# Gabriel-SGama/Semantic-SuperPoint

Hardware: NVIDIA B200
Metric: loss-step pairs/s @240x320 B32 (higher is better)
Workload: dtype bf16x3 (hi/lo split bf16 on tcgen05, fp32 accumulate, fp32-grade)

## Files before the change

include/ssp_b200.h:

```cpp
#ifndef SSP_B200_H
#define SSP_B200_H
#include <stddef.h>
#include <stdint.h>
#ifdef __cplusplus
extern "C" {
#endif

int ssp_version(void);
const char* ssp_last_error(void);
int ssp_sm_count(void);

int ssp_warp_points(const float* pts , int P, const float* H , int B,
                    float* out , void* stream);
int ssp_warp_points_mask(const float* pts, int P, const float* H, int B, float shape_x, float shape_y,
                         float* out , uint8_t* keep , void* stream);
int ssp_warp_keypoints_f64(const double* kp , int K, const double* H , double W,
                           double Hh, double* out , uint8_t* keep , void* stream);

int ssp_inv_warp_image(const float* img , int B, int C, int H, int W, const float* Hinv ,
                       const float* xs, const float* ys, int mode, float* out , void* stream);

int ssp_valid_mask(int B, int H, int W, const float* Hinv, const float* xs, const float* ys, const uint8_t* kern,
                   int kh, int kw, int ax, int ay, float* out , void* stream);

int ssp_labels2d_to_3d(const float* labels , int B, int H, int W, int add_dustbin,
                       float* out , void* stream);
int ssp_cell_mask(const float* mask2d , int B, int H, int W, float* out , void* stream);
size_t ssp_detector_loss_ws_bytes(int B, int Hc, int Wc);
int ssp_detector_loss_fwd(const float* semi , const float* target, const float* mask, int B, int Hc,
                          int Wc, int fused2d, float* out3, void* ws, size_t ws_bytes, void* stream);
int ssp_detector_loss_bwd(const float* semi, const float* target, const float* mask, int B, int Hc, int Wc,
                          int fused2d, const float* fwd_out3, const float* gout , float* dsemi, void* stream);
int ssp_detector_loss_fwd_pair(const float* semi0, const float* target0, const float* mask0, const float* semi1,
                               const float* target1, const float* mask1, int B, int Hc, int Wc, int fused2d,
                               float* out3_0, float* out3_1, float* cellmask1, void* ws, size_t ws_bytes, void* stream);
int ssp_detector_loss_bwd_pair(const float* semi0, const float* target0, const float* mask0, const float* semi1,
                               const float* target1, const float* mask1, int B, int Hc, int Wc, int fused2d,
                               const float* fwd0, const float* fwd1, const float* gout0, const float* gout1,
                               float* dsemi0, float* dsemi1, void* stream);

int ssp_flatten_detection(const float* semi , int N, int Hc, int Wc, float* heat ,
                          void* stream);

int ssp_flatten_detection_masked(const float* semi , const float* mask , int N, int Hc,
                                 int Wc, float* heat , int* flag, void* stream);

int ssp_combine_heatmap(const float* heat , const float* mask ,
                        const float* Hinv , int I, int N, int H, int W, const float* xs, const float* ys,
                        float* out , void* stream);
int ssp_combine_heatmap_signed(const float* heat_signed , const float* Hinv , int I, int N, int H,
                               int W, const float* xs, const float* ys, const int* flag , float* out ,
                               void* stream);

size_t ssp_nms_ws_bytes(int I, int H, int W, int capacity);
int ssp_nms_fast(const float* heat , int I, int H, int W, float conf_thresh, int R, const uint8_t* stencil,
                 int border, int capacity, double* pts, int* counts_host, void* ws, size_t ws_bytes, void* stream);
int ssp_box_nms(const float* prob , int I, int H, int W, float min_prob, int R, const uint8_t* stencil,
                float* out , void* ws, size_t ws_bytes, void* stream);

int ssp_desc_geometry_nblocks(int B, int Nc);
int ssp_desc_geometry(const float* H , const float* mask_valid ,
                      const float* mask2d , int B,
                      int Hc, int Wc, int cell, float* wpts, float* mv_pad, double* mv_part ,
                      uint32_t* mvbits , void* stream);
int ssp_desc_pos_nblocks(int B, int Nc);
int ssp_desc_maxp(void);
int ssp_desc_pos_fwd(const float* D , const float* Dw, const float* wpts, const float* mv_pad, int B,
                     int Hc, int Wc, int Dch, int cell, float dist, float lamda, float mpos, float mneg,
                     double* partials, int* rowcol, float* rowdot, int* colcnt, int* colrow, float* coldot,
                     void* stream);
int ssp_desc_pos_planes_nblocks(int B, int Nc);
int ssp_desc_pos_fwd_planes(const void* Ahi, const void* Alo, const void* Bhi, const void* Blo, const float* wpts,
                            const float* mv_pad, int B, int Hc, int Wc, int cell, float dist, float lamda, float mpos,
                            float mneg, double* partials, int* rowcol, float* rowdot, int* colcnt, int* colrow,
                            float* coldot, void* stream);
int ssp_desc_dense_simt_nblocks(int B, int Nc);
int ssp_desc_dense_fwd_simt(const float* D, const float* Dw, const float* mv_pad, int B, int Hc, int Wc, int Dch,
                            float mneg, double* partials, uint32_t* bitsR, uint32_t* bitsC,
                            float* dbgS , void* stream);
int ssp_desc_pack(const float* src , const float* scale , int B, int Dch, int Nc,
                  void* hi , void* lo , void* stream);
int ssp_desc_pack2(const float* src0, const float* src1 , const float* scale, int B, int Dch, int Nc, void* hi0,
                   void* lo0, void* hi1, void* lo1, void* stream);
int ssp_desc_pack2_geometry(const float* src0, const float* src1, int B, int Dch, int Hc, int Wc, void* hi0, void* lo0 ,
                            void* hi1, void* lo1 , const float* H , const float* mask_valid ,
                            const float* mask2d , int cell, float* wpts, float* mv_pad, double* mv_part,
                            uint32_t* mvbits , void* stream);
int ssp_desc_dense_tc_nblocks(int B, int Nc);
int ssp_desc_dense_fwd_tc(const void* Ahi, const void* Alo, const void* Bhi, const void* Blo, const float* mv_pad,
                          const uint32_t* mvbits , int B, int Hc, int Wc, float mneg, double* partials,
                          uint32_t* bitsR, uint32_t* bitsC, float* dbgS, void* stream);
int ssp_desc_finalize(const double* pos_part, int npos, const double* neg_part, int nneg, const double* mv_part,
                      int nmv, int B, int Hc, int Wc, const int* overflow, float* out8,
                      const float* det0 , const float* det1, float lambda_loss, float* total , void* stream);
int ssp_desc_pair_mask(const float* wpts, int B, int Hc, int Wc, int cell, float dist, float* mask ,
                       void* stream);
int ssp_desc_alpha(const float* mv_pad, const float* g3 , const float* out8, int B,
                   int Nc_pad, float* alpha , float* srow ,
                   void* stream);
int ssp_desc_pos_coef(const int* rowcol, const float* rowdot, const int* colcnt, const int* colrow, const float* coldot,
                      const uint32_t* bitsR, const float* mv_pad, const float* g3, float gscale, int gmode,
                      const float* out8, int B, int Nc_pad, float lamda, float mpos, float* rowcoef, int* colrow_sorted,
                      float* colcoef, float* alpha_out, float* srow_out, uint32_t* bitsC_out, int Nc, void* stream);
int ssp_step_bwd_prologue(const float* semi0, const float* labels0, const float* mask0, const float* semi1,
                          const float* labels1, const float* mask1, int B, int Hc, int Wc, const float* fwd0 ,
                          const float* fwd1, const float* gout , float* dsemi0, float* dsemi1,
                          const int* rowcol, const float* rowdot, const int* colcnt, const int* colrow, const float* coldot,
                          const uint32_t* bitsR, const float* mv_pad, const float* g3, float gscale, int gmode,
                          const float* out8, float lamda, float mpos, float* rowcoef, int* colrow_sorted, float* colcoef,
                          float* alpha_out, float* srow_out, uint32_t* bitsC_out, void* stream);
int ssp_desc_pos_apply(const int* rowcol, const float* rowcoef, const int* colrow, const float* colcoef, const float* D,
                       const float* Dw, int B, int Dch, int Nc, int which , float* dD, float* dDw,
                       void* stream);
int ssp_desc_bits_gemm_simt(const uint32_t* bits, const float* src , const float* colscale,
                            const float* rowscale, const int* plist, const float* pcoef, const float* possrc, int B,
                            int Dch, int Nc, float* out , void* stream);
int ssp_desc_bits_gemm_tc_planes(const uint32_t* bits, const void* Bhi, const void* Blo, const float* rowscale,
                                 const int* plist, const float* pcoef, const void* pos_hi, const void* pos_lo, int B,
                                 int Nc, float* out , void* stream);
int ssp_desc_bits_gemm_tc_pair(const uint32_t* bits0, const void* Bhi0, const void* Blo0, const float* rowscale0,
                               const int* plist0, const float* pcoef0, const void* pos_hi0, const void* pos_lo0,
                               float* out0, const uint32_t* bits1, const void* Bhi1, const void* Blo1,
                               const float* rowscale1, const int* plist1, const float* pcoef1, const void* pos_hi1,
                               const void* pos_lo1, float* out1, int B, int Nc, void* stream);

size_t ssp_sem_ce_ws_bytes(int B, int C, int H, int W, int upsampled);
int ssp_sem_ce_fwd(const float* logits , const long long* labels, int B, int C, int H, int W,
                   int ignore_index, float* lse2 ,
                   float* out3, void* ws, size_t ws_bytes, void* stream);
int ssp_sem_ce_bwd(const float* logits, const long long* labels, const float* lse2, int B, int C, int H, int W,
                   int ignore_index, const float* out3, const float* gout ,
                   float* dlogits , void* stream);
int ssp_sem_ce_up8(const float* logits_lr, const long long* labels, int B, int C, int Hc, int Wc, int ignore_index,
                   float* gsum, float* out3, void* ws, size_t ws_bytes, void* stream);
int ssp_sem_ce_up8_bwd(const float* gsum, const float* out3, const float* gout, int B, int C, int Hc, int Wc,
                       float* dlogits , void* stream);

int ssp_sample_desc(const float* coarse, const double* pts, int K, int D, int Hc, int Wc, int cell, float* desc,
                    void* stream);
int ssp_nn_match(const float* desc1 , const float* desc2 , int D, int K1, int K2,
                 unsigned long long* best1 , unsigned long long* best2 , void* stream);

int ssp_transpose_batched(const float* src , int B, int rows, int cols, float* dst ,
                          void* stream);
int ssp_sparse_desc_loss_fwd(const float* Dt, const float* Dwt, const int* ia, const int* ib, int B, int Nc, int Dch, int K,
                             int Kn, float lamda, float mpos, float mneg, float* dots, float* stats, float* out3,
                             void* stream);
int ssp_sparse_desc_loss_bwd(const float* Dt, const float* Dwt, const int* ia, const int* ib, const float* dots,
                             const float* stats, const float* g3 , int B, int Nc, int Dch, int K, int Kn,
                             float lamda, float mpos, float mneg, float* dDt, float* dDwt, void* stream);
int ssp_sparse_sample(const float* mat_H , int B, int Hc, int Wc, int K, int nper, unsigned long long* state,
                      int* ia, int* ib, int* M , void* stream);
int ssp_sparse_finalize(const int* M , int B, float* out3, const float* det0, const float* det1,
                        float lambda_loss, float* total , void* stream);

size_t ssp_warp_labels_ws_bytes(int B, int H, int W);
int ssp_warp_labels(const float* pnts, const int* counts, int B, int Pmax, int H, int W, const float* Hpix, int bilinear,
                    float* labels, float* res, float* labels_bi , float* warped, int* kept, void* ws,
                    size_t ws_bytes, void* stream);

size_t ssp_xchg_bytes(void);
int ssp_xchg_max_ranks(void);
int ssp_xchg_alloc(void** buf, void* ipc_handle64_host);
int ssp_xchg_open(const void* ipc_handle64_host, void** peer_buf);
int ssp_xchg_close(void* peer_buf);
int ssp_xchg_free(void* buf);
int ssp_xchg_status(const void* local_buf, void* stream);
int ssp_loss_exchange(const void* const* bufs_host , int rank, int world,
                      float* det0, float* det1, float* desc8, float* sem0, float* sem1, int B_local, int Hc, int Wc,
                      float lambda_loss, float* total ,
                      double timeout_s, void* stream);

int ssp_debug_trace(void* buf);
int ssp_debug_trace_cap(void);

#ifdef __cplusplus
}
#endif
#endif
```

semantic-superpoint_b200/_lib.py:

```python
import ctypes
import os
import threading

import torch

from . import build as _build

_c = ctypes
_P = _c.c_void_p
_I = _c.c_int
_F = _c.c_float
_D = _c.c_double
_Z = _c.c_size_t

SIGNATURES = {
    "ssp_version": (_I, []),
    "ssp_last_error": (_c.c_char_p, []),
    "ssp_sm_count": (_I, []),
    "ssp_warp_points": (_I, [_P, _I, _P, _I, _P, _P]),
    "ssp_warp_points_mask": (_I, [_P, _I, _P, _I, _F, _F, _P, _P, _P]),
    "ssp_warp_keypoints_f64": (_I, [_P, _I, _P, _D, _D, _P, _P, _P]),
    "ssp_inv_warp_image": (_I, [_P, _I, _I, _I, _I, _P, _P, _P, _I, _P, _P]),
    "ssp_valid_mask": (_I, [_I, _I, _I, _P, _P, _P, _P, _I, _I, _I, _I, _P, _P]),
    "ssp_labels2d_to_3d": (_I, [_P, _I, _I, _I, _I, _P, _P]),
    "ssp_cell_mask": (_I, [_P, _I, _I, _I, _P, _P]),
    "ssp_detector_loss_ws_bytes": (_Z, [_I, _I, _I]),
    "ssp_detector_loss_fwd": (_I, [_P, _P, _P, _I, _I, _I, _I, _P, _P, _Z, _P]),
    "ssp_detector_loss_bwd": (_I, [_P, _P, _P, _I, _I, _I, _I, _P, _P, _P, _P]),
    "ssp_detector_loss_fwd_pair": (_I, [_P, _P, _P, _P, _P, _P, _I, _I, _I, _I, _P, _P, _P, _P, _Z, _P]),
    "ssp_detector_loss_bwd_pair": (_I, [_P, _P, _P, _P, _P, _P, _I, _I, _I, _I, _P, _P, _P, _P, _P, _P, _P]),
    "ssp_flatten_detection": (_I, [_P, _I, _I, _I, _P, _P]),
    "ssp_flatten_detection_masked": (_I, [_P, _P, _I, _I, _I, _P, _P, _P]),
    "ssp_combine_heatmap": (_I, [_P, _P, _P, _I, _I, _I, _I, _P, _P, _P, _P]),
    "ssp_combine_heatmap_signed": (_I, [_P, _P, _I, _I, _I, _I, _P, _P, _P, _P, _P]),
    "ssp_nms_ws_bytes": (_Z, [_I, _I, _I, _I]),
    "ssp_nms_fast": (_I, [_P, _I, _I, _I, _F, _I, _P, _I, _I, _P, _P, _P, _Z, _P]),
    "ssp_box_nms": (_I, [_P, _I, _I, _I, _F, _I, _P, _P, _P, _Z, _P]),
    "ssp_desc_geometry_nblocks": (_I, [_I, _I]),
    "ssp_desc_geometry": (_I, [_P, _P, _P, _I, _I, _I, _I, _P, _P, _P, _P, _P]),
    "ssp_desc_pos_nblocks": (_I, [_I, _I]),
    "ssp_desc_maxp": (_I, []),
    "ssp_desc_pos_fwd": (_I, [_P, _P, _P, _P, _I, _I, _I, _I, _I, _F, _F, _F, _F, _P, _P, _P, _P, _P, _P, _P]),
    "ssp_desc_pos_planes_nblocks": (_I, [_I, _I]),
    "ssp_desc_pos_fwd_planes": (_I, [_P, _P, _P, _P, _P, _P, _I, _I, _I, _I, _F, _F, _F, _F, _P, _P, _P, _P, _P, _P, _P]),
    "ssp_desc_dense_simt_nblocks": (_I, [_I, _I]),
    "ssp_desc_dense_fwd_simt": (_I, [_P, _P, _P, _I, _I, _I, _I, _F, _P, _P, _P, _P, _P]),
    "ssp_desc_pack": (_I, [_P, _P, _I, _I, _I, _P, _P, _P]),
    "ssp_desc_pack2": (_I, [_P, _P, _P, _I, _I, _I, _P, _P, _P, _P, _P]),
    "ssp_desc_pack2_geometry": (_I, [_P, _P, _I, _I, _I, _I, _P, _P, _P, _P, _P, _P, _P, _I, _P, _P, _P, _P, _P]),
    "ssp_desc_dense_tc_nblocks": (_I, [_I, _I]),
    "ssp_desc_dense_fwd_tc": (_I, [_P, _P, _P, _P, _P, _P, _I, _I, _I, _F, _P, _P, _P, _P, _P]),
    "ssp_desc_finalize": (_I, [_P, _I, _P, _I, _P, _I, _I, _I, _I, _P, _P, _P, _P, _F, _P, _P]),
    "ssp_desc_pair_mask": (_I, [_P, _I, _I, _I, _I, _F, _P, _P]),
    "ssp_desc_alpha": (_I, [_P, _P, _P, _I, _I, _P, _P, _P]),
    "ssp_desc_pos_coef": (_I, [_P, _P, _P, _P, _P, _P, _P, _P, _F, _I, _P, _I, _I, _F, _F, _P, _P, _P, _P, _P, _P, _I, _P]),
    "ssp_step_bwd_prologue": (_I, [_P] * 6 + [_I] * 3 + [_P] * 5 + [_P] * 8 + [_F, _I, _P, _F, _F] + [_P] * 7),
    "ssp_desc_pos_apply": (_I, [_P, _P, _P, _P, _P, _P, _I, _I, _I, _I, _P, _P, _P]),
    "ssp_desc_bits_gemm_simt": (_I, [_P, _P, _P, _P, _P, _P, _P, _I, _I, _I, _P, _P]),
    "ssp_desc_bits_gemm_tc_planes": (_I, [_P, _P, _P, _P, _P, _P, _P, _P, _I, _I, _P, _P]),
    "ssp_desc_bits_gemm_tc_pair": (_I, [_P] * 18 + [_I, _I, _P]),
    "ssp_sem_ce_ws_bytes": (_Z, [_I, _I, _I, _I, _I]),
    "ssp_sem_ce_fwd": (_I, [_P, _P, _I, _I, _I, _I, _I, _P, _P, _P, _Z, _P]),
    "ssp_sem_ce_bwd": (_I, [_P, _P, _P, _I, _I, _I, _I, _I, _P, _P, _P, _P]),
    "ssp_sem_ce_up8": (_I, [_P, _P, _I, _I, _I, _I, _I, _P, _P, _P, _Z, _P]),
    "ssp_sem_ce_up8_bwd": (_I, [_P, _P, _P, _I, _I, _I, _I, _P, _P]),
    "ssp_sample_desc": (_I, [_P, _P, _I, _I, _I, _I, _I, _P, _P]),
    "ssp_nn_match": (_I, [_P, _P, _I, _I, _I, _P, _P, _P]),
    "ssp_transpose_batched": (_I, [_P, _I, _I, _I, _P, _P]),
    "ssp_sparse_desc_loss_fwd": (_I, [_P, _P, _P, _P, _I, _I, _I, _I, _I, _F, _F, _F, _P, _P, _P, _P]),
    "ssp_sparse_desc_loss_bwd": (_I, [_P, _P, _P, _P, _P, _P, _P, _I, _I, _I, _I, _I, _F, _F, _F, _P, _P, _P]),
    "ssp_sparse_sample": (_I, [_P, _I, _I, _I, _I, _I, _P, _P, _P, _P, _P]),
    "ssp_sparse_finalize": (_I, [_P, _I, _P, _P, _P, _F, _P, _P]),
    "ssp_warp_labels_ws_bytes": (_Z, [_I, _I, _I]),
    "ssp_warp_labels": (_I, [_P, _P, _I, _I, _I, _I, _P, _I, _P, _P, _P, _P, _P, _P, _Z, _P]),
    "ssp_debug_trace": (_I, [_P]),
    "ssp_debug_trace_cap": (_I, []),
    "ssp_xchg_bytes": (_Z, []),
    "ssp_xchg_max_ranks": (_I, []),
    "ssp_xchg_alloc": (_I, [_c.POINTER(_P), _P]),
    "ssp_xchg_open": (_I, [_P, _c.POINTER(_P)]),
    "ssp_xchg_close": (_I, [_P]),
    "ssp_xchg_free": (_I, [_P]),
    "ssp_xchg_status": (_I, [_P, _P]),
    "ssp_loss_exchange": (_I, [_c.POINTER(_P), _I, _I, _P, _P, _P, _P, _P, _I, _I, _I, _F, _P, _D, _P]),
}

_lib = None
_lock = threading.Lock()
launch_count = 0


def lib_path():
    return _build.LIB_PATH


def load(build_if_missing=True):
    global _lib
    with _lock:
        if _lib is not None:
            return _lib
        path = _build.LIB_PATH
        if not os.path.exists(path):
            if not build_if_missing:
                raise RuntimeError("libssp_b200.so is missing: run `python -c 'import __graft_entry__ as g; g.build()'`")
            _build.build_library()
        lib = ctypes.CDLL(path)
        for name, (res, args) in SIGNATURES.items():
            fn = getattr(lib, name)
            fn.restype = res
            fn.argtypes = args
        _lib = lib
        return _lib


def check(rc, what):
    if rc != 0:
        msg = load().ssp_last_error()
        raise RuntimeError("%s failed (code %d): %s" % (what, rc, msg.decode() if msg else ""))


KERNELS_PER_CALL = {"ssp_nms_fast": 5, "ssp_box_nms": 4, "ssp_detector_loss_fwd": 2, "ssp_detector_loss_fwd_pair": 2,
                    "ssp_sem_ce_fwd": 2, "ssp_sem_ce_up8": 2}
kernel_count = 0
_prof = None


def profile_begin():
    global _prof
    _prof = {}


def profile_end():
    global _prof
    torch.cuda.synchronize()
    out = {k: (len(v), sum(a.elapsed_time(b) for a, b in v)) for k, v in _prof.items()}
    _prof = None
    return out


def call(name, *args):
    global launch_count, kernel_count
    launch_count += 1
    kernel_count += KERNELS_PER_CALL.get(name, 1)
    fn = getattr(load(), name)
    if _prof is None:
        check(fn(*args), name)
        return
    e0, e1 = torch.cuda.Event(enable_timing=True), torch.cuda.Event(enable_timing=True)
    e0.record()
    rc = fn(*args)
    e1.record()
    _prof.setdefault(name, []).append((e0, e1))
    check(rc, name)


def ptr(t):
    return None if t is None else _c.c_void_p(t.data_ptr())


def stream_of(t):
    return _c.c_void_p(torch.cuda.current_stream(t.device).cuda_stream)


def require_cuda(*tensors):
    for t in tensors:
        if t is not None and not t.is_cuda:
            raise RuntimeError(
                "ssp_b200 has no CPU path: got a %s tensor; move inputs to a CUDA device (sm_100a)" % t.device
            )


def f32c(t, device=None):
    if device is not None and t.device != torch.device(device):
        t = t.to(device)
    if t.dtype != torch.float32:
        t = t.float()
    t = t.contiguous()
    if t.data_ptr() % 16:
        t = t.clone()
    return t
```

semantic-superpoint_b200/csrc/desc_tc.cu:

```cuda
#include "desc_common.cuh"
#include "tc_ptx.cuh"
#include <algorithm>
#include <cstdlib>

#define TRACE_CAP 4096
#ifdef SSP_TRACE
__device__ long long* g_trace_buf = nullptr;
__device__ int g_trace_roles = 0xF;
#define TR_DECL(role) long long* tr_ = (g_trace_buf && ((g_trace_roles >> (role)) & 1)) ? g_trace_buf + ((size_t)blockIdx.x * 4 + (role)) * TRACE_CAP : nullptr; int trn_ = 0
#define TR_ONLY(cond) do { if (!(cond)) tr_ = nullptr; } while (0)
#define TR(tag) do { if (tr_ && trn_ < TRACE_CAP) tr_[trn_++] = (clock64() << 8) | (long long)(tag); } while (0)
#else
#define TR_DECL(role) do { } while (0)
#define TR_ONLY(cond) do { } while (0)
#define TR(tag) do { } while (0)
#endif

namespace {

constexpr int BM = 128;
constexpr int BN = 256;
constexpr int KD = 256;
constexpr int KC = 64;
constexpr int NKC = KD / KC;
constexpr int CHUNK_BYTES = BM * KC * 2;
constexpr int FWD_THREADS = 320;
constexpr int BAR_BYTES = 1024;

template <int P> struct FwdCfg {
  static constexpr int A_BYTES = P * NKC * CHUNK_BYTES;
  static constexpr int STAGE_BYTES = P * CHUNK_BYTES;
  static constexpr int NSTAGE = (P == 1) ? 10 : 3;
  static constexpr int B_BYTES = NSTAGE * STAGE_BYTES;
  static constexpr int SMEM = A_BYTES + B_BYTES + BAR_BYTES + 1024;
};

__device__ __forceinline__ uint8_t* align1024(uint8_t* p) {
  return reinterpret_cast<uint8_t*>((reinterpret_cast<uintptr_t>(p) + 1023) & ~(uintptr_t)1023);
}

template <bool BITS>
__device__ __forceinline__ void epi_chunk(const uint32_t (&v)[32], const float4 (&mq)[8], float mneg, uint64_t& su2,
                                          uint64_t& sw2, uint32_t& rowword) {
  const uint64_t mneg2 = tc::pack2(mneg, mneg);
  uint32_t eb[32];
#pragma unroll
  for (int i = 0; i < 16; ++i) {
    const uint64_t e2 = tc::sub2(mneg2, tc::pack2(__uint_as_float(v[2 * i]), __uint_as_float(v[2 * i + 1])));
    float e0, e1;
    tc::unpack2(e2, e0, e1);
    const uint64_t n2 = tc::pack2(fmaxf(-e0, 0.f), fmaxf(-e1, 0.f));
    su2 = tc::add2(su2, n2);
    const float4 m = mq[i >> 1];
    sw2 = tc::fma2(n2, (i & 1) ? tc::pack2(m.z, m.w) : tc::pack2(m.x, m.y), sw2);
    eb[2 * i] = __float_as_uint(e0);
    eb[2 * i + 1] = __float_as_uint(e1);
  }
  if (BITS) {
    uint32_t w = 0;
#pragma unroll
    for (int pos = 31; pos >= 0; --pos) {
      const int j = ((pos & 15) << 1) | (pos >> 4);
      w = __funnelshift_l(eb[j], w, 1);
    }
    rowword = w;
  }
}

__device__ __forceinline__ double f32_to_f64_bits(float f) {
  const uint32_t u = __float_as_uint(f);
  const uint32_t e = (u >> 23) & 0xffu;
  const unsigned long long sign = (unsigned long long)(u & 0x80000000u) << 32;
  unsigned long long d;
  if (e == 0u) d = sign;
  else if (e == 0xffu) d = sign | (0x7ffull << 52) | ((unsigned long long)(u & 0x7fffffu) << 29);
  else d = sign | ((unsigned long long)(e + 896u) << 52) | ((unsigned long long)(u & 0x7fffffu) << 29);
  return __longlong_as_double((long long)d);
}

template <int P, bool BITS>
__global__ void __launch_bounds__(FWD_THREADS, 1)
desc_dense_fwd_tc_kernel(const __grid_constant__ CUtensorMap tmA, const __grid_constant__ CUtensorMap tmB,
                         const __grid_constant__ CUtensorMap tmBl, const float* __restrict__ mv_pad, const uint32_t* __restrict__ mvbits, DescGeom g, int n_last,
                         double* __restrict__ partials, uint32_t* __restrict__ bitsR, float* __restrict__ dbgS) {
  using Cfg = FwdCfg<P>;
  constexpr int NSTAGE = Cfg::NSTAGE;
  extern __shared__ uint8_t smem_raw[];
  uint8_t* smem = align1024(smem_raw);
  uint8_t* sA = smem;
  uint8_t* sB = sA + Cfg::A_BYTES;
  uint64_t* bars = reinterpret_cast<uint64_t*>(sB + Cfg::B_BYTES);
  uint64_t* a_full = bars;
  uint64_t* a_empty = a_full + NKC;
  uint64_t* b_full = a_empty + NKC;
  uint64_t* b_empty = b_full + NSTAGE;
  uint64_t* t_full = b_empty + NSTAGE;
  uint64_t* t_empty = t_full + 2;
  uint32_t* tmem_ptr = reinterpret_cast<uint32_t*>(t_empty + 2);

  const int warp = threadIdx.x >> 5, lane = threadIdx.x & 31;
  const int MP = g.Nc_pad / (2 * BM), NT = g.Nc_pad / BN;
  const uint32_t cta_rank = tc::cluster_ctarank();
  const bool leader = cta_rank == 0;
  const int ncluster = gridDim.x >> 1, cid = blockIdx.x >> 1;
  const long long T = (long long)g.B * MP * NT;
  const int it0 = (int)(T * cid / ncluster), it1 = (int)(T * (cid + 1) / ncluster);

  if (warp == 8 && lane == 0) {
    tc::prefetch_tmap(&tmA);
    tc::prefetch_tmap(&tmB);
    tc::prefetch_tmap(&tmBl);
  }
  if (warp == 9) {
    if (lane == 0) {
      for (int k = 0; k < NKC; ++k) { tc::mbar_init(a_full + k, 1); tc::mbar_init(a_empty + k, 1); }
      for (int s = 0; s < NSTAGE; ++s) { tc::mbar_init(b_full + s, 1); tc::mbar_init(b_empty + s, 1); }
      for (int s = 0; s < 2; ++s) { tc::mbar_init(t_full + s, 1); tc::mbar_init(t_empty + s, 16); }
      tc::fence_barrier_init();
    }
    __syncwarp();
    tc::tmem_alloc2(tmem_ptr, 512);
  }
  tc::fence_before_sync();
  tc::cluster_sync_all();
  tc::fence_after_sync();
  const uint32_t tmem_base = *tmem_ptr;

  if (warp == 8) {
    {
      TR_DECL(1);
      TR_ONLY(lane == 0);
      const bool el = tc::elect_one();
      int prev_key = -1, stage_it = 0, nkeys = 0;
      for (int it = it0; it < it1; ++it) {
        const int key = it / NT, nt = it - key * NT;
        const int b = key / MP, mp = key - b * MP;
        const int row_base = b * g.Nc_pad;
        const bool newkey = key != prev_key;
        const bool last = nt == NT - 1;
        const int half = (last ? n_last : BN) >> 1;
        for (int kc = 0; kc < NKC; ++kc) {
          if (newkey) {
            TR(10);
            if (nkeys > 0) tc::mbar_wait(a_empty + kc, (uint32_t)((nkeys - 1) & 1));
            TR(11);
            if (el) {
              if (leader) tc::mbar_expect_tx(a_full + kc, 2 * P * CHUNK_BYTES);
              tc::tma_load_3d_2sm(&tmA, a_full + kc, sA + kc * P * CHUNK_BYTES, kc * KC, row_base + (2 * mp + (int)cta_rank) * BM, 0);
            }
          }
          {
            const int s = stage_it % NSTAGE;
            const uint32_t ph = (stage_it / NSTAGE) & 1;
            ++stage_it;
            TR(12);
            tc::mbar_wait(b_empty + s, ph ^ 1);
            TR(13);
            if (el) {
              if (leader) tc::mbar_expect_tx(b_full + s, 2 * P * half * KC * 2);
              tc::tma_load_3d_2sm(last ? &tmBl : &tmB, b_full + s, sB + s * Cfg::STAGE_BYTES, kc * KC,
                                  row_base + nt * BN + (int)cta_rank * half, 0);
            }
          }
        }
        if (newkey) { prev_key = key; ++nkeys; }
      }
    }
    __syncwarp();
  } else if (warp == 9) {
    if (leader) {
      TR_DECL(0);
      TR_ONLY(lane == 0);
      const bool el = tc::elect_one();
      if (tmem_base != 0u) __trap();
      const uint32_t sA_u = tc::smem_u32(sA), sB_u = tc::smem_u32(sB);
      int prev_key = -1, stage_it = 0, tcount = 0, nkeys = 0;
      for (int it = it0; it < it1; ++it, ++tcount) {
        const int key = it / NT, nt = it - key * NT;
        const bool newkey = key != prev_key;
        if (newkey) { prev_key = key; ++nkeys; }
        const bool last_of_key = (it + 1 == it1) || ((it + 1) / NT != key);
        const int ncols = nt == NT - 1 ? n_last : BN;
        const uint32_t idesc = tc::idesc_bf16_f32(2 * BM, ncols, 0, 0);
        const int as = tcount & 1;
        const uint32_t aph = (tcount >> 1) & 1;
        TR(2);
        tc::mbar_wait(t_empty + as, aph ^ 1);
        TR(3);
        tc::fence_after_sync();
        const uint32_t d_tmem = as * BN;
        uint32_t first = 1;
        for (int kc = 0; kc < NKC; ++kc) {
          if (newkey) {
            TR(1);
            tc::mbar_wait(a_full + kc, (uint32_t)((nkeys - 1) & 1));
            TR(8);
          }
          {
            const int s = stage_it % NSTAGE;
            const uint32_t ph = (stage_it / NSTAGE) & 1;
            ++stage_it;
            TR(4);
            tc::mbar_wait(b_full + s, ph);
            TR(5);
            tc::fence_after_sync();
            const uint64_t da_hi = tc::smem_desc_sw128(sA_u + (kc * P) * CHUNK_BYTES, 16, 1024);
            const uint64_t db_hi = tc::smem_desc_sw128(sB_u + s * Cfg::STAGE_BYTES, 16, 1024);
            if (el) {
              tc::mma2_ss_x4(d_tmem, da_hi, db_hi, idesc, first ? 0u : 1u);
              if (P == 2) {
                const uint64_t da_lo = tc::smem_desc_sw128(sA_u + (kc * P + 1) * CHUNK_BYTES, 16, 1024);
                const uint64_t db_lo = tc::smem_desc_sw128(sB_u + s * Cfg::STAGE_BYTES + (ncols >> 1) * (KC * 2), 16, 1024);
                tc::mma2_ss_x4(d_tmem, da_lo, db_hi, idesc, 1u);
                tc::mma2_ss_x4(d_tmem, da_hi, db_lo, idesc, 1u);
              }
              tc::mma2_commit_mc(b_empty + s, (uint16_t)0x3);
            }
            first = 0;
            TR(6);
          }
          if (last_of_key && el) tc::mma2_commit_mc(a_empty + kc, (uint16_t)0x3);
        }
        if (el) tc::mma2_commit_mc(t_full + as, (uint16_t)0x3);
        __syncwarp();
      }
    }
    __syncwarp();
  } else {
    const int q = warp & 3, half = warp >> 2;
    const int NW = g.Nc_pad / 32;
    const bool fold = mvbits != nullptr;
    int tcount = 0;
    double su_all = 0.0, sw_all = 0.0;
    TR_DECL(2 + (warp == 7 ? 1 : 0));
    TR_ONLY((warp == 0 || warp == 7) && lane == 0);
    for (int it = it0; it < it1; ++it, ++tcount) {
      const int key = it / NT, nt = it - key * NT;
      const int b = key / MP, mp = key - b * MP;
      const int row_base = b * g.Nc_pad;
      const int m0 = (2 * mp + (int)cta_rank) * BM;
      const int row = m0 + q * 32 + lane;
      const int ncols = nt == NT - 1 ? n_last : BN;
      const int ch0 = half * 4, ch1 = min((ncols + 31) >> 5, ch0 + 4);
      const int as = tcount & 1;
      const uint32_t aph = (tcount >> 1) & 1;
      float4 mq[8];
      if (ch0 < ch1) {
        const float4* mvq = reinterpret_cast<const float4*>(mv_pad + (size_t)row_base + nt * BN + ch0 * 32);
#pragma unroll
        for (int j4 = 0; j4 < 8; ++j4) mq[j4] = __ldg(mvq + j4);
      }
      TR(30);
      tc::mbar_wait(t_full + as, aph);
      TR(31);
      tc::fence_after_sync();
      uint64_t su2 = 0ull, sw2 = 0ull;
#pragma unroll 1
      for (int ch = ch0; ch < ch1; ++ch) {
        const int cbase = nt * BN + ch * 32;
        uint32_t v[32];
        tc::tmem_ld32(tmem_base + ((uint32_t)(q * 32) << 16) + as * BN + ch * 32, v);
        float4 mnext[8];
        if (ch + 1 < ch1) {
          const float4* mvq = reinterpret_cast<const float4*>(mv_pad + (size_t)row_base + cbase + 32);
#pragma unroll
          for (int j4 = 0; j4 < 8; ++j4) mnext[j4] = __ldg(mvq + j4);
        }
        tc::tmem_ld_wait();
        if (ch * 32 + 32 > ncols) {
#pragma unroll
          for (int j = 16; j < 32; ++j) v[j] = 0u;
        }
        uint32_t rowword = 0;
        epi_chunk<BITS>(v, mq, g.mneg, su2, sw2, rowword);
        if (BITS) {
          if (fold) rowword &= __ldg(mvbits + (size_t)b * NW + cbase / 32);
          bitsR[((size_t)b * NW + cbase / 32) * g.Nc_pad + row] = rowword;
        }
        if (dbgS && row < g.Nc) {
#pragma unroll
          for (int j = 0; j < 32; ++j)
            if (cbase + j < g.Nc) dbgS[((size_t)b * g.Nc + row) * g.Nc + cbase + j] = __uint_as_float(v[j]);
        }
        if (ch + 1 < ch1) {
#pragma unroll
          for (int j4 = 0; j4 < 8; ++j4) mq[j4] = mnext[j4];
        }
      }
      tc::fence_before_sync();
      __syncwarp();
      if (lane == 0) tc::mbar_arrive_leader(t_empty + as);
      TR(32);
      float sa, sb, wa, wb;
      tc::unpack2(su2, sa, sb);
      tc::unpack2(sw2, wa, wb);
      su_all += f32_to_f64_bits(sa + sb);
      sw_all += f32_to_f64_bits(wa + wb);
    }
    su_all = warp_sum_d(su_all);
    sw_all = warp_sum_d(sw_all);
    if (lane == 0) {
      const size_t slot = ((size_t)blockIdx.x * 8 + warp) * 2;
      partials[slot] = su_all;
      partials[slot + 1] = sw_all;
    }
  }

  tc::fence_before_sync();
  tc::cluster_sync_all();
  if (warp == 9) {
    tc::fence_after_sync();
    tc::tmem_dealloc2(tmem_base, 512);
  }
}

__global__ void __launch_bounds__(256)
desc_bits_transpose_kernel(const uint32_t* __restrict__ bitsR, uint32_t* __restrict__ bitsC, int NW, int NWv, int Nc_pad) {
  const int lane = threadIdx.x & 31, warp = threadIdx.x >> 5;
  const int rw = blockIdx.x, b = blockIdx.y;
  const int rl = ((lane & 15) << 1) | (lane >> 4);
  for (int cw0 = warp; cw0 < NW; cw0 += 32) {
    uint32_t w[4];
#pragma unroll
    for (int u = 0; u < 4; ++u) {
      const int cw = cw0 + 8 * u;
      w[u] = (cw < NWv && rw < NWv) ? __ldg(bitsR + ((size_t)b * NW + cw) * Nc_pad + rw * 32 + rl) : 0u;
    }
#pragma unroll
    for (int u = 0; u < 4; ++u) {
      const int cw = cw0 + 8 * u;
      if (cw >= NW) break;
      bitsC[((size_t)b * NW + rw) * Nc_pad + cw * 32 + rl] = warp_transpose32(w[u], lane);
    }
  }
}

constexpr int KT = 128;
constexpr int BG_PLANE_BYTES = KT * 128;
constexpr int BG_N = 128;
constexpr int BG_THREADS = 576;
constexpr int BG_W_EPI = 8, BG_W_TMA = 16, BG_W_MMA = 17;
constexpr int BG_NS = 4;
constexpr int BG_ACOLS = KT / 2;

constexpr int BG_PF = 4;
constexpr int BG_WRING_BYTES = 2 * BG_PF * 4 * BM * 4;

template <int P> struct BgCfg {
  static constexpr int STAGE_BYTES = P * BG_PLANE_BYTES;
  static constexpr int SMEM = BG_NS * STAGE_BYTES + BAR_BYTES + BG_WRING_BYTES + 1024;
};

struct BgJob {
  const uint32_t* bits;
  const float* rowscale;
  const int* plist;
  const float* pcoef;
  const uint4* pos_hi;
  const uint4* pos_lo;
  float* out;
};

template <int P>
__global__ void __launch_bounds__(BG_THREADS, 1)
desc_bits_gemm_tc_kernel(const __grid_constant__ CUtensorMap tm0, const __grid_constant__ CUtensorMap tm1, BgJob job0,
                         BgJob job1, int njobs, int B, int Nc, int Nc_pad) {
  using Cfg = BgCfg<P>;
  constexpr int NS = BG_NS;
  static_assert(256 + BG_ACOLS * NS <= 512, "TMEM A ring does not fit");
  extern __shared__ uint8_t smem_raw[];
  uint8_t* smem = align1024(smem_raw);
  uint64_t* bars = reinterpret_cast<uint64_t*>(smem + NS * Cfg::STAGE_BYTES);
  uint64_t* b_full = bars;
  uint64_t* a_full = b_full + NS;
  uint64_t* s_free = a_full + NS;
  uint64_t* d_full = s_free + NS;
  uint64_t* d_empty = d_full + 2;
  uint32_t* tmem_ptr = reinterpret_cast<uint32_t*>(d_empty + 2);
  uint32_t* wring = reinterpret_cast<uint32_t*>(smem + NS * Cfg::STAGE_BYTES + BAR_BYTES);

  const int warp = threadIdx.x >> 5, lane = threadIdx.x & 31;
  const int MP = Nc_pad / (2 * BM), NK = (Nc + KT - 1) / KT, NW = Nc_pad / 32;
  const int NKS = (Nc + 15) / 16;
  const uint32_t cta_rank = tc::cluster_ctarank();
  const bool leader = cta_rank == 0;
  const int ncluster = gridDim.x >> 1, cid = blockIdx.x >> 1;
  const int T = B * njobs * MP * 2;
  constexpr uint32_t A_COL0 = 256;

  auto decode = [&](int it, int& b, int& jb, int& mp, int& dh) {
    dh = it & 1;
    int t = it >> 1;
    mp = t % MP;
    t /= MP;
    jb = t % njobs;
    b = t / njobs;
  };

  if (warp == BG_W_TMA && lane == 0) {
    tc::prefetch_tmap(&tm0);
    if (njobs > 1) tc::prefetch_tmap(&tm1);
  }
  if (warp == BG_W_MMA) {
    if (lane == 0) {
      for (int s = 0; s < NS; ++s) { tc::mbar_init(b_full + s, 1); tc::mbar_init(a_full + s, 8); tc::mbar_init(s_free + s, 1); }
      for (int s = 0; s < 2; ++s) { tc::mbar_init(d_full + s, 1); tc::mbar_init(d_empty + s, 16); }
      tc::fence_barrier_init();
    }
    __syncwarp();
    tc::tmem_alloc2(tmem_ptr, 512);
  }
  tc::fence_before_sync();
  tc::cluster_sync_all();
  tc::fence_after_sync();
  const uint32_t tmem_base = *tmem_ptr;

  if (warp == BG_W_TMA) {
    {
      TR_DECL(1);
      TR_ONLY(lane == 0);
      const bool el = tc::elect_one();
      int st_it = 0;
      for (int it = cid; it < T; it += ncluster) {
        int b, jb, mp, dh;
        decode(it, b, jb, mp, dh);
        const CUtensorMap* m = jb ? &tm1 : &tm0;
        for (int kc = 0; kc < NK; ++kc, ++st_it) {
          const int s = st_it % NS;
          const uint32_t ph = (st_it / NS) & 1;
          TR(12);
          tc::mbar_wait(s_free + s, ph ^ 1);
          TR(13);
          if (el) {
            if (leader) tc::mbar_expect_tx(b_full + s, 2 * Cfg::STAGE_BYTES);
            tc::tma_load_3d_2sm(m, b_full + s, smem + s * Cfg::STAGE_BYTES, dh * BG_N + (int)cta_rank * 64, b * Nc_pad + kc * KT, 0);
          }
        }
      }
    }
    __syncwarp();
  } else if (warp == BG_W_MMA) {
    if (leader) {
      TR_DECL(0);
      TR_ONLY(lane == 0);
      const bool el = tc::elect_one();
      if (tmem_base != 0u) __trap();
      constexpr uint32_t idesc = tc::idesc_bf16_f32(2 * BM, BG_N, 0, 1);
      const uint32_t smem_u = tc::smem_u32(smem);
      int st_it = 0, tcount = 0;
      for (int it = cid; it < T; it += ncluster, ++tcount) {
        const int as = tcount & 1;
        const uint32_t aph = (tcount >> 1) & 1;
        TR(2);
        tc::mbar_wait(d_empty + as, aph ^ 1);
        TR(3);
        tc::fence_after_sync();
        const uint32_t d_tmem = as * BG_N;
        uint32_t first = 1;
        for (int kc = 0; kc < NK; ++kc, ++st_it) {
          const int s = st_it % NS;
          const uint32_t ph = (st_it / NS) & 1;
          TR(4);
          tc::mbar_wait(b_full + s, ph);
          TR(5);
          tc::mbar_wait(a_full + s, ph);
          TR(7);
          tc::fence_after_sync();
          const int nks = min(KT / 16, NKS - kc * (KT / 16));
          for (int p = 0; p < P; ++p) {
            const uint64_t db = tc::smem_desc_sw128(smem_u + s * Cfg::STAGE_BYTES + p * BG_PLANE_BYTES, BG_PLANE_BYTES, 1024);
            for (int j = 0; j < nks; ++j) {
              if (el) tc::mma2_ts(d_tmem, A_COL0 + s * BG_ACOLS + 8 * j, db + (uint64_t)(128 * j), idesc, first ? 0u : 1u);
              first = 0;
            }
          }
          if (el) tc::mma2_commit_mc(s_free + s, (uint16_t)0x3);
          TR(6);
        }
        if (el) tc::mma2_commit_mc(d_full + as, (uint16_t)0x3);
        __syncwarp();
      }
    }
    __syncwarp();
  } else if (warp < BG_W_EPI) {
    const int q = warp & 3, set = warp >> 2;
    TR_DECL(2);
    TR_ONLY(warp == 0 && lane == 0);
    auto expand_words = [&](uint32_t w0, uint32_t w1, uint32_t (&r)[32]) {
#pragma unroll
      for (int i = 0; i < 15; ++i) {
        r[i] = (w0 << (14 - i)) & 0x40004000u;
        r[16 + i] = (w1 << (14 - i)) & 0x40004000u;
      }
      r[15] = (w0 >> 1) & 0x40004000u;
      r[31] = (w1 >> 1) & 0x40004000u;
    };
    auto expand_stage = [&](int st_it, const uint32_t (&w)[4]) {
      const int s = st_it % NS;
      const uint32_t ph = (st_it / NS) & 1;
      uint32_t r[32];
      expand_words(w[0], w[1], r);
      TR(20);
      tc::mbar_wait(s_free + s, ph ^ 1);
      TR(21);
      tc::fence_after_sync();
      const uint32_t t0 = tmem_base + ((uint32_t)(q * 32) << 16) + A_COL0 + s * BG_ACOLS;
      tc::tmem_st32(t0, r);
      expand_words(w[2], w[3], r);
      tc::tmem_st32(t0 + 32, r);
      tc::tmem_st_wait();
      tc::fence_before_sync();
      __syncwarp();
      if (lane == 0) tc::mbar_arrive_leader(a_full + s);
      TR(23);
    };
    constexpr int PF = BG_PF;
    uint32_t* myring = wring + (size_t)set * PF * 4 * BM + (q * 32 + lane);
    int itB = cid, kcB = set;
    const uint32_t* pB = nullptr;
    bool newitem = true;
    auto fetch = [&](int slot) {
      while (itB < T && kcB >= NK) { kcB -= NK; itB += ncluster; newitem = true; }
      if (itB < T) {
        if (newitem) {
          int b, jb, mp, dh;
          decode(itB, b, jb, mp, dh);
          const int row = (2 * mp + (int)cta_rank) * BM + q * 32 + lane;
          pB = (jb ? job1.bits : job0.bits) + (size_t)b * NW * Nc_pad + row;
          newitem = false;
        }
#pragma unroll
        for (int u = 0; u < 4; ++u) tc::cp_async4(myring + (slot * 4 + u) * BM, pB + (size_t)(4 * kcB + u) * Nc_pad);
        kcB += 2;
      }
      tc::cp_async_commit();
    };
#pragma unroll
    for (int u = 0; u < PF; ++u) fetch(u);
    const int nitems = cid < T ? (T - cid + ncluster - 1) / ncluster : 0;
    const int total = nitems * NK;
    for (int g0 = set; g0 < total; g0 += 2 * PF) {
#pragma unroll
      for (int u = 0; u < PF; ++u) {
        if (g0 + 2 * u < total) {
          tc::cp_async_wait<PF - 1>();
          uint32_t w[4];
#pragma unroll
          for (int v = 0; v < 4; ++v) w[v] = myring[(u * 4 + v) * BM];
          expand_stage(g0 + 2 * u, w);
          fetch(u);
        }
      }
    }
    tc::cp_async_wait<0>();
  } else {
    const int q = warp & 3, chalf = (warp - BG_W_EPI) >> 2;
    int tcount = 0;
    TR_DECL(3);
    TR_ONLY(warp == BG_W_EPI && lane == 0);
    for (int it = cid; it < T; it += ncluster, ++tcount) {
      int b, jb, mp, dh;
      decode(it, b, jb, mp, dh);
      const BgJob& J = jb ? job1 : job0;
      const int row = (2 * mp + (int)cta_rank) * BM + q * 32 + lane;
      const bool row_ok = row < Nc;
      float rs = 0.5f;
      if (J.rowscale && row_ok) rs *= J.rowscale[(size_t)b * Nc_pad + row];
      const int* pl = J.plist ? J.plist + ((size_t)b * Nc_pad + row) * DESC_MAXP : nullptr;
      const float* pcf = J.plist ? J.pcoef + ((size_t)b * Nc_pad + row) * DESC_MAXP : nullptr;
      int npos = 0;
      if (pl && row_ok) {
#pragma unroll
        for (int n = 0; n < DESC_MAXP; ++n)
          if (pl[n] >= 0) npos = n + 1;
      }
      const int nmax = __reduce_max_sync(0xffffffffu, npos);
      const int as = tcount & 1;
      const uint32_t aph = (tcount >> 1) & 1;
      TR(30);
      tc::mbar_wait(d_full + as, aph);
      TR(31);
      tc::fence_after_sync();
      auto add_partner = [&](int n, int ch, float (&val)[32]) {
        int pc = n < npos ? pl[n] : -1;
        if (pc < 0) return;
        float pf = pcf[n];
        const size_t o = (((size_t)b * Nc_pad + pc) * KD + dh * BG_N + ch * 32) >> 3;
#pragma unroll
        for (int u = 0; u < 4; ++u) {
          const uint4 h = __ldg(J.pos_hi + o + u);
          const uint32_t hw[4] = {h.x, h.y, h.z, h.w};
          uint32_t lw[4] = {0u, 0u, 0u, 0u};
          if (J.pos_lo) {
            const uint4 l = __ldg(J.pos_lo + o + u);
            lw[0] = l.x; lw[1] = l.y; lw[2] = l.z; lw[3] = l.w;
          }
#pragma unroll
          for (int i = 0; i < 4; ++i) {
            float e0 = __uint_as_float(hw[i] << 16) + __uint_as_float(lw[i] << 16);
            float e1 = __uint_as_float(hw[i] & 0xffff0000u) + __uint_as_float(lw[i] & 0xffff0000u);
            val[u * 8 + 2 * i] = fmaf(pf, e0, val[u * 8 + 2 * i]);
            val[u * 8 + 2 * i + 1] = fmaf(pf, e1, val[u * 8 + 2 * i + 1]);
          }
        }
      };
#pragma unroll 1
      for (int ch = chalf * 2; ch < chalf * 2 + 2; ++ch) {
        uint32_t v[32];
        tc::tmem_ld32(tmem_base + ((uint32_t)(q * 32) << 16) + as * BG_N + ch * 32, v);
        tc::tmem_ld_wait();
        if (row_ok) {
          float val[32];
#pragma unroll
          for (int j = 0; j < 32; ++j) val[j] = __uint_as_float(v[j]) * rs;
#pragma unroll 1
          for (int n = 0; n < nmax; ++n) add_partner(n, ch, val);
          float* o = J.out + ((size_t)b * KD + dh * BG_N + ch * 32) * Nc + row;
#pragma unroll
          for (int j = 0; j < 32; ++j) o[(size_t)j * Nc] = val[j];
        }
      }
      tc::fence_before_sync();
      __syncwarp();
      if (lane == 0) tc::mbar_arrive_leader(d_empty + as);
      TR(32);
    }
  }

  tc::fence_before_sync();
  tc::cluster_sync_all();
  if (warp == BG_W_MMA) {
    tc::fence_after_sync();
    tc::tmem_dealloc2(tmem_base, 512);
  }
}

typedef CUresult (*EncodeTiledFn)(CUtensorMap*, CUtensorMapDataType, cuuint32_t, void*, const cuuint64_t*,
                                  const cuuint64_t*, const cuuint32_t*, const cuuint32_t*, CUtensorMapInterleave,
                                  CUtensorMapSwizzle, CUtensorMapL2promotion, CUtensorMapFloatOOBfill);

EncodeTiledFn get_encode_tiled() {
  static EncodeTiledFn fn = nullptr;
  if (!fn) {
    void* p = nullptr;
    cudaDriverEntryPointQueryResult qres;
    if (cudaGetDriverEntryPoint("cuTensorMapEncodeTiled", &p, cudaEnableDefault, &qres) == cudaSuccess &&
        qres == cudaDriverEntryPointSuccess)
      fn = reinterpret_cast<EncodeTiledFn>(p);
  }
  return fn;
}

int make_planes_map3(CUtensorMap* m, const void* hi, const void* lo, uint64_t rows, uint32_t box_rows) {
  EncodeTiledFn enc = get_encode_tiled();
  if (!enc) { ssp_set_error("cuTensorMapEncodeTiled unavailable (driver too old?)"); return SSP_EUNSUPPORTED; }
  const uint64_t plane_bytes = rows * KD * 2;
  uint64_t pstride = plane_bytes;
  if (lo) {
    if ((uintptr_t)lo <= (uintptr_t)hi || (((uintptr_t)lo - (uintptr_t)hi) & 15) || ((uintptr_t)lo - (uintptr_t)hi) < plane_bytes ||
        ((uintptr_t)lo - (uintptr_t)hi) >= (1ull << 40)) {
      ssp_set_error("tcgen05 descriptor kernels: the lo plane must lie above the hi plane (distance a multiple of 16 bytes)");
      return SSP_EARG;
    }
    pstride = (uintptr_t)lo - (uintptr_t)hi;
  }
  cuuint64_t dims[3] = {(cuuint64_t)KD, (cuuint64_t)rows, (cuuint64_t)(lo ? 2 : 1)};
  cuuint64_t strides[2] = {(cuuint64_t)KD * 2, (cuuint64_t)pstride};
  cuuint32_t box[3] = {(cuuint32_t)KC, box_rows, (cuuint32_t)(lo ? 2 : 1)};
  cuuint32_t estr[3] = {1, 1, 1};
  CUresult r = enc(m, CU_TENSOR_MAP_DATA_TYPE_BFLOAT16, 3, const_cast<void*>(hi), dims, strides, box, estr,
                   CU_TENSOR_MAP_INTERLEAVE_NONE, CU_TENSOR_MAP_SWIZZLE_128B, CU_TENSOR_MAP_L2_PROMOTION_L2_256B,
                   CU_TENSOR_MAP_FLOAT_OOB_FILL_NONE);
  if (r != CUDA_SUCCESS) { ssp_set_error("cuTensorMapEncodeTiled (3-D planes) failed with CUresult %d", (int)r); return SSP_EARG; }
  return SSP_OK;
}

template <typename... KArgs, typename... Args>
int launch_cluster2(void (*kernel)(KArgs...), int grid, int block, int smem, cudaStream_t st, Args... args) {
  cudaLaunchConfig_t cfg = {};
  cfg.gridDim = dim3(grid);
  cfg.blockDim = dim3(block);
  cfg.dynamicSmemBytes = smem;
  cfg.stream = st;
  cudaLaunchAttribute attr[1];
  attr[0].id = cudaLaunchAttributeClusterDimension;
  attr[0].val.clusterDim.x = 2;
  attr[0].val.clusterDim.y = 1;
  attr[0].val.clusterDim.z = 1;
  cfg.attrs = attr;
  cfg.numAttrs = 1;
  cudaError_t e = cudaLaunchKernelEx(&cfg, kernel, args...);
  if (e != cudaSuccess) { ssp_set_error("cluster launch failed: %s", cudaGetErrorString(e)); return (int)e; }
  return SSP_OK;
}

template <typename K>
int set_smem(K kernel, int bytes) {
  cudaError_t e = cudaFuncSetAttribute(kernel, cudaFuncAttributeMaxDynamicSharedMemorySize, bytes);
  if (e != cudaSuccess) { ssp_set_error("cudaFuncSetAttribute(%d B smem) failed: %s", bytes, cudaGetErrorString(e)); return (int)e; }
  return SSP_OK;
}

}

extern "C" int ssp_debug_trace(void* buf) {
#ifdef SSP_TRACE
  long long* p = reinterpret_cast<long long*>(buf);
  SSP_CUDA_CALL(cudaMemcpyToSymbol(g_trace_buf, &p, sizeof(p)));
  const char* e = getenv("SSP_TRACE_ROLES");
  int roles = e ? atoi(e) : 0xF;
  SSP_CUDA_CALL(cudaMemcpyToSymbol(g_trace_roles, &roles, sizeof(roles)));
  return SSP_OK;
#else
  (void)buf;
  ssp_set_error("ssp_debug_trace: library built without -DSSP_TRACE");
  return SSP_EUNSUPPORTED;
#endif
}
extern "C" int ssp_debug_trace_cap(void) { return TRACE_CAP; }

extern "C" int ssp_desc_dense_tc_nblocks(int B, int Nc) {
  int ncp = desc_nc_pad(Nc);
  long long items = (long long)B * (ncp / (2 * BM)) * (ncp / BN);
  int nclusters = (int)std::min<long long>(items, std::max(1, ssp_num_sms() / 2));
  return 2 * nclusters * 8;
}

extern "C" int ssp_desc_dense_fwd_tc(const void* Ahi, const void* Alo, const void* Bhi, const void* Blo,
                                     const float* mv_pad, const uint32_t* mvbits, int B, int Hc, int Wc, float mneg,
                                     double* partials, uint32_t* bitsR, uint32_t* bitsC, float* dbgS, void* stream) {
  SSP_REQUIRE(Ahi && Bhi && mv_pad && partials, "ssp_desc_dense_fwd_tc: null pointer");
  SSP_REQUIRE((Alo == nullptr) == (Blo == nullptr), "ssp_desc_dense_fwd_tc: lo planes must both be given or both null");
  SSP_REQUIRE(!bitsC || bitsR, "ssp_desc_dense_fwd_tc: bitsC needs bitsR");
  SSP_REQUIRE(B > 0 && B <= 65535 && Hc > 0 && Wc > 0, "ssp_desc_dense_fwd_tc: bad sizes");
  SSP_REQUIRE(mneg > 0.f, "ssp_desc_dense_fwd_tc: margin_neg must be > 0 (zero padding relies on it)");
  SSP_REQUIRE((((uintptr_t)Ahi | (uintptr_t)Bhi | (uintptr_t)Alo | (uintptr_t)Blo | (uintptr_t)mv_pad) & 15) == 0,
              "ssp_desc_dense_fwd_tc: operands must be 16-byte aligned");
  DescGeom g;
  g.B = B; g.Hc = Hc; g.Wc = Wc; g.Nc = Hc * Wc; g.Nc_pad = desc_nc_pad(g.Nc); g.Dch = KD;
  g.cell = 0; g.dist = 0.f; g.lamda = 0.f; g.mpos = 0.f; g.mneg = mneg;
  const int NT = g.Nc_pad / BN;
  const int n_last = ((g.Nc - (NT - 1) * BN) + 15) / 16 * 16;
  uint64_t rows = (uint64_t)B * g.Nc_pad;
  CUtensorMap mA, mB, mL;
  int rc;
  if ((rc = make_planes_map3(&mA, Ahi, Alo, rows, BM))) return rc;
  if ((rc = make_planes_map3(&mB, Bhi, Blo, rows, BN / 2))) return rc;
  if ((rc = make_planes_map3(&mL, Bhi, Blo, rows, n_last / 2))) return rc;
  long long items = (long long)B * (g.Nc_pad / (2 * BM)) * NT;
  int nclusters = (int)std::min<long long>(items, std::max(1, ssp_num_sms() / 2));
  int grid = 2 * nclusters;
  cudaStream_t st = (cudaStream_t)stream;
#define LAUNCH_FWD(PP, BB)                                                                                       \
  do {                                                                                                           \
    if ((rc = set_smem(desc_dense_fwd_tc_kernel<PP, BB>, FwdCfg<PP>::SMEM))) return rc;                          \
    if ((rc = launch_cluster2(desc_dense_fwd_tc_kernel<PP, BB>, grid, FWD_THREADS, FwdCfg<PP>::SMEM, st, mA, mB, mL,         \
                              mv_pad, mvbits, g, n_last, partials, bitsR, dbgS))) return rc;                     \
  } while (0)
  if (Alo) { if (bitsR) LAUNCH_FWD(2, true); else LAUNCH_FWD(2, false); }
  else     { if (bitsR) LAUNCH_FWD(1, true); else LAUNCH_FWD(1, false); }
#undef LAUNCH_FWD
  SSP_CUDA_CHECK_LAUNCH("desc_dense_fwd_tc_kernel");
  if (bitsC) {
    const int NW = g.Nc_pad / 32, NWv = (g.Nc + 31) / 32;
    dim3 tg(NW, B);
    desc_bits_transpose_kernel<<<tg, 256, 0, st>>>(bitsR, bitsC, NW, NWv, g.Nc_pad);
    SSP_CUDA_CHECK_LAUNCH("desc_bits_transpose_kernel");
  }
  return SSP_OK;
}

struct BgHostJob {
  const uint32_t* bits; const void* Bhi; const void* Blo; const float* rowscale; const int* plist; const float* pcoef;
  const void* pos_hi; const void* pos_lo; float* out;
};

static int bits_gemm_tc_launch(const BgHostJob* jobs, int njobs, int B, int Nc, void* stream) {
  SSP_REQUIRE(B > 0 && Nc > 0, "ssp_desc_bits_gemm_tc: bad sizes");
  int Nc_pad = desc_nc_pad(Nc);
  uint64_t rows = (uint64_t)B * Nc_pad;
  CUtensorMap maps[2];
  BgJob dj[2] = {};
  int rc;
  for (int j = 0; j < njobs; ++j) {
    const BgHostJob& h = jobs[j];
    SSP_REQUIRE(h.bits && h.Bhi && h.out, "ssp_desc_bits_gemm_tc: null pointer");
    SSP_REQUIRE(!h.plist || (h.pcoef && h.pos_hi), "ssp_desc_bits_gemm_tc: plist needs pcoef and the partner planes");
    SSP_REQUIRE((((uintptr_t)h.Bhi | (uintptr_t)h.Blo | (uintptr_t)h.pos_hi | (uintptr_t)h.pos_lo) & 15) == 0,
                "ssp_desc_bits_gemm_tc: operands must be 16-byte aligned");
    SSP_REQUIRE((h.Blo == nullptr) == (jobs[0].Blo == nullptr), "ssp_desc_bits_gemm_tc: both jobs must use the same engine (lo planes)");
    if ((rc = make_planes_map3(&maps[j], h.Bhi, h.Blo, rows, KT))) return rc;
    dj[j].bits = h.bits; dj[j].rowscale = h.rowscale; dj[j].plist = h.plist; dj[j].pcoef = h.pcoef;
    dj[j].pos_hi = (const uint4*)h.pos_hi; dj[j].pos_lo = (const uint4*)h.pos_lo; dj[j].out = h.out;
  }
  if (njobs == 1) { maps[1] = maps[0]; dj[1] = dj[0]; }
  long long items = (long long)B * njobs * (Nc_pad / (2 * BM)) * 2;
  int nclusters = (int)std::min<long long>(items, std::max(1, ssp_num_sms() / 2));
  int grid = 2 * nclusters;
  cudaStream_t st = (cudaStream_t)stream;
  if (jobs[0].Blo) {
    if ((rc = set_smem(desc_bits_gemm_tc_kernel<2>, BgCfg<2>::SMEM))) return rc;
    if ((rc = launch_cluster2(desc_bits_gemm_tc_kernel<2>, grid, BG_THREADS, BgCfg<2>::SMEM, st, maps[0], maps[1], dj[0], dj[1], njobs,
                              B, Nc, Nc_pad))) return rc;
  } else {
    if ((rc = set_smem(desc_bits_gemm_tc_kernel<1>, BgCfg<1>::SMEM))) return rc;
    if ((rc = launch_cluster2(desc_bits_gemm_tc_kernel<1>, grid, BG_THREADS, BgCfg<1>::SMEM, st, maps[0], maps[1], dj[0], dj[1], njobs,
                              B, Nc, Nc_pad))) return rc;
  }
  SSP_CUDA_CHECK_LAUNCH("desc_bits_gemm_tc_kernel");
  return SSP_OK;
}

extern "C" int ssp_desc_bits_gemm_tc_planes(const uint32_t* bits, const void* Bhi, const void* Blo, const float* rowscale,
                                            const int* plist, const float* pcoef, const void* pos_hi, const void* pos_lo,
                                            int B, int Nc, float* out, void* stream) {
  BgHostJob j = {bits, Bhi, Blo, rowscale, plist, pcoef, pos_hi, pos_lo, out};
  return bits_gemm_tc_launch(&j, 1, B, Nc, stream);
}

extern "C" int ssp_desc_bits_gemm_tc_pair(const uint32_t* bits0, const void* Bhi0, const void* Blo0, const float* rowscale0,
                                          const int* plist0, const float* pcoef0, const void* pos_hi0, const void* pos_lo0,
                                          float* out0, const uint32_t* bits1, const void* Bhi1, const void* Blo1,
                                          const float* rowscale1, const int* plist1, const float* pcoef1, const void* pos_hi1,
                                          const void* pos_lo1, float* out1, int B, int Nc, void* stream) {
  BgHostJob j[2] = {{bits0, Bhi0, Blo0, rowscale0, plist0, pcoef0, pos_hi0, pos_lo0, out0},
                    {bits1, Bhi1, Blo1, rowscale1, plist1, pcoef1, pos_hi1, pos_lo1, out1}};
  return bits_gemm_tc_launch(j, 2, B, Nc, stream);
}
```

semantic-superpoint_b200/losses.py:

```python
import torch
from torch.autograd.function import once_differentiable

from . import _lib
from ._lib import call, f32c, ptr, stream_of

_ENGINES = ("bf16x3", "bf16", "fp32")
_engine = "bf16x3"
CHECK_LIST_OVERFLOW = False


def set_descriptor_engine(name):
    global _engine
    if name not in _ENGINES:
        raise ValueError("descriptor engine must be one of %s" % (_ENGINES,))
    _engine = name


def get_descriptor_engine():
    return _engine


_side_streams = {}
_SAME = object()


class _Fork(object):

    def __init__(self, dev):
        self.cur = torch.cuda.current_stream(dev)
        key = (dev.index, self.cur.cuda_stream)
        if key not in _side_streams:
            _side_streams[key] = torch.cuda.Stream(device=dev)
        self.side = _side_streams[key]
        self.ctx = None

    def __enter__(self):
        self.side.wait_stream(self.cur)
        self.ctx = torch.cuda.stream(self.side)
        self.ctx.__enter__()
        return self

    def __exit__(self, *exc):
        self.ctx.__exit__(*exc)
        return False

    def join(self):
        self.cur.wait_stream(self.side)


class DetectorLossFn(torch.autograd.Function):

    @staticmethod
    def forward(ctx, semi, target, mask, fused2d, dist_group=None):
        _lib.require_cuda(semi)
        dev = semi.device
        x = f32c(semi.detach(), dev)
        t = f32c(target.detach(), dev)
        m = f32c(mask.detach(), dev)
        B, C, Hc, Wc = x.shape
        if C != 65:
            raise RuntimeError("detector_loss: input must have 65 channels, got %d" % C)
        if fused2d:
            if t.numel() != B * Hc * Wc * 64 or m.numel() != B * Hc * Wc * 64:
                raise RuntimeError("detector_loss_2d: labels_2D / mask_2D must be [B,1,8Hc,8Wc]")
        else:
            if t.shape != x.shape or m.numel() != B * Hc * Wc:
                raise RuntimeError("detector_loss: target must be [B,65,Hc,Wc] and mask [B,Hc,Wc]")
        out3 = torch.empty((3,), dtype=torch.float32, device=dev)
        nbytes = _lib.load().ssp_detector_loss_ws_bytes(B, Hc, Wc)
        ws = torch.empty((nbytes,), dtype=torch.uint8, device=dev)
        call("ssp_detector_loss_fwd", ptr(x), ptr(t), ptr(m), B, Hc, Wc, 1 if fused2d else 0, ptr(out3), ptr(ws),
             nbytes, stream_of(x))
        ctx.save_for_backward(x, t, m)
        ctx.out3 = out3
        ctx.fused2d = fused2d
        if dist_group is not None:
            from .dist import globalize_detector
            globalize_detector(out3, dist_group)
        return out3[0]

    @staticmethod
    @once_differentiable
    def backward(ctx, gout):
        x, t, m = ctx.saved_tensors
        out3 = ctx.out3
        B, C, Hc, Wc = x.shape
        g = f32c(gout.reshape(1), x.device)
        dsemi = torch.empty_like(x)
        call("ssp_detector_loss_bwd", ptr(x), ptr(t), ptr(m), B, Hc, Wc, 1 if ctx.fused2d else 0, ptr(out3), ptr(g),
             ptr(dsemi), stream_of(x))
        return dsemi, None, None, None, None


class SemanticLossFn(torch.autograd.Function):

    @staticmethod
    def forward(ctx, pred, label, ignore_index, dist_group=None):
        _lib.require_cuda(pred)
        dev = pred.device
        x = f32c(pred.detach(), dev)
        lab = label.detach().to(device=dev, dtype=torch.int64).contiguous()
        if x.dim() != 4 or lab.dim() != 3 or lab.shape[0] != x.shape[0]:
            raise RuntimeError("sem_loss: expected pred [B,C,h,w] and label [B,H,W], got %s and %s"
                               % (tuple(pred.shape), tuple(label.shape)))
        B, C, h, w = x.shape
        H, W = lab.shape[1:]
        up = (h, w) != (H, W)
        if up and (H != 8 * h or W != 8 * w):
            raise RuntimeError("sem_loss: pred %dx%d must match the label size %dx%d or be exactly 1/8 of it" % (h, w, H, W))
        out3 = torch.empty((3,), dtype=torch.float32, device=dev)
        nbytes = _lib.load().ssp_sem_ce_ws_bytes(B, C, H, W, 1 if up else 0)
        ws = torch.empty((nbytes,), dtype=torch.uint8, device=dev)
        need_grad = ctx.needs_input_grad[0]
        if up:
            gsum = torch.empty_like(x) if need_grad else None
            call("ssp_sem_ce_up8", ptr(x), ptr(lab), B, C, h, w, int(ignore_index), ptr(gsum), ptr(out3), ptr(ws), nbytes,
                 stream_of(x))
            ctx.saved = (gsum,)
        else:
            lse2 = torch.empty((B, H, W), dtype=torch.float32, device=dev)
            call("ssp_sem_ce_fwd", ptr(x), ptr(lab), B, C, H, W, int(ignore_index), ptr(lse2), ptr(out3), ptr(ws), nbytes,
                 stream_of(x))
            ctx.saved = (x, lab, lse2)
        ctx.up, ctx.shape, ctx.ignore = up, (B, C, h, w), int(ignore_index)
        ctx.out3 = out3
        if dist_group is not None:
            from .dist import globalize_semantic
            globalize_semantic(out3, dist_group)
        return out3[0]

    @staticmethod
    @once_differentiable
    def backward(ctx, gout):
        B, C, h, w = ctx.shape
        out3 = ctx.out3
        g = f32c(gout.reshape(1), out3.device)
        if ctx.up:
            (gsum,) = ctx.saved
            d = torch.empty_like(gsum)
            call("ssp_sem_ce_up8_bwd", ptr(gsum), ptr(out3), ptr(g), B, C, h, w, ptr(d), stream_of(d))
        else:
            x, lab, lse2 = ctx.saved
            d = torch.empty_like(x)
            call("ssp_sem_ce_bwd", ptr(x), ptr(lab), ptr(lse2), B, C, h, w, ctx.ignore, ptr(out3), ptr(g), ptr(d),
                 stream_of(d))
        return d, None, None, None


class DetectorLossPairFn(torch.autograd.Function):

    @staticmethod
    def forward(ctx, semi, target, mask, semi_w, target_w, mask_w, fused2d, dist_group=None):
        _lib.require_cuda(semi, semi_w)
        dev = semi.device
        x0, t0, m0 = f32c(semi.detach(), dev), f32c(target.detach(), dev), f32c(mask.detach(), dev)
        x1, t1, m1 = f32c(semi_w.detach(), dev), f32c(target_w.detach(), dev), f32c(mask_w.detach(), dev)
        B, C, Hc, Wc = x0.shape
        if C != 65 or x1.shape != x0.shape:
            raise RuntimeError("detector_loss: inputs must be two [B,65,Hc,Wc] tensors of the same shape")
        n2d = B * Hc * Wc * 64
        for t, m in ((t0, m0), (t1, m1)):
            ok = (t.numel() == n2d and m.numel() == n2d) if fused2d else (t.shape == x0.shape and m.numel() == B * Hc * Wc)
            if not ok:
                raise RuntimeError("detector_loss: target / mask shapes do not match the logits")
        out = torch.empty((2, 3), dtype=torch.float32, device=dev)
        cellmask = torch.empty((B, Hc, Wc), dtype=torch.float32, device=dev)
        per = (_lib.load().ssp_detector_loss_ws_bytes(B, Hc, Wc) + 15) // 16 * 16
        ws = torch.empty((2 * per,), dtype=torch.uint8, device=dev)
        call("ssp_detector_loss_fwd_pair", ptr(x0), ptr(t0), ptr(m0), ptr(x1), ptr(t1), ptr(m1), B, Hc, Wc,
             1 if fused2d else 0, ptr(out[0]), ptr(out[1]), ptr(cellmask), ptr(ws), 2 * per, stream_of(x0))
        ctx.save_for_backward(x0, t0, m0, x1, t1, m1)
        ctx.out = out
        ctx.fused2d = fused2d
        ctx.mark_non_differentiable(cellmask)
        if dist_group is not None:
            from .dist import get_exchange
            get_exchange(dist_group).run(det0=out[0], det1=out[1])
        return out[0, 0], out[1, 0], cellmask

    @staticmethod
    @once_differentiable
    def backward(ctx, g0, g1, _gm):
        x0, t0, m0, x1, t1, m1 = ctx.saved_tensors
        out = ctx.out
        B, C, Hc, Wc = x0.shape
        dev = x0.device
        if g1 is _SAME:
            g = f32c(g0.reshape(1), dev).expand(2)
        else:
            zero = torch.zeros((), dtype=torch.float32, device=dev)
            g = torch.stack([(a if a is not None else zero).reshape(()).to(torch.float32) for a in (g0, g1)]).contiguous()
        d0, d1 = torch.empty_like(x0), torch.empty_like(x1)
        call("ssp_detector_loss_bwd_pair", ptr(x0), ptr(t0), ptr(m0), ptr(x1), ptr(t1), ptr(m1), B, Hc, Wc,
             1 if ctx.fused2d else 0, ptr(out[0]), ptr(out[1]), ptr(g[0:1]), ptr(g[1:2]) if g1 is not _SAME else ptr(g[0:1]),
             ptr(d0), ptr(d1), stream_of(x0))
        return d0, None, None, d1, None, None, None, None


def _nc_pad(nc):
    return (nc + 255) // 256 * 256


class DescriptorLossFn(torch.autograd.Function):

    @staticmethod
    def forward(ctx, D, Dw, Hm, mv, cell, lamda, dist, engine, dist_group=None, debug_S=None, fold_alpha=False, step_total=None):
        lib = _lib.load()
        dev = D.device
        Dc = f32c(D.detach(), dev)
        Dwc = f32c(Dw.detach(), dev)
        if Dc.shape != Dwc.shape:
            raise RuntimeError("descriptor_loss: descriptor shapes differ")
        B, Dch, Hc, Wc = Dc.shape
        Nc = Hc * Wc
        Ncp = _nc_pad(Nc)
        st = stream_of(Dc)
        mpos, mneg = 1.0, 0.2
        if engine not in _ENGINES:
            raise ValueError("descriptor engine must be one of %s" % (_ENGINES,))
        if Dch != 256:
            engine = "fp32"
        need_grad = bool(ctx.needs_input_grad[0] or ctx.needs_input_grad[1])
        split = engine == "bf16x3"
        fold_alpha = bool(fold_alpha and need_grad and engine != "fp32")

        wpts = torch.empty((B, Ncp, 2), dtype=torch.float32, device=dev)
        mv_pad = torch.empty((B, Ncp), dtype=torch.float32, device=dev)
        mvbits = torch.empty((B, Ncp // 32), dtype=torch.int32, device=dev) if fold_alpha else None
        nmv = lib.ssp_desc_geometry_nblocks(B, Nc)
        mv_part = torch.empty((nmv,), dtype=torch.float64, device=dev)
        mask2d = None
        if isinstance(mv, tuple):
            mask2d, mv = mv[1], None
        geom_args = (ptr(Hm), ptr(mv), ptr(mask2d), cell, ptr(wpts), ptr(mv_pad), ptr(mv_part), ptr(mvbits))
        if engine == "fp32":
            call("ssp_desc_geometry", geom_args[0], geom_args[1], geom_args[2], B, Hc, Wc, *geom_args[3:], st)

        maxp = lib.ssp_desc_maxp()
        npos = lib.ssp_desc_pos_planes_nblocks(B, Nc) if split else lib.ssp_desc_pos_nblocks(B, Nc)
        pos_part = torch.empty((npos, 4), dtype=torch.float64, device=dev)
        lists_i = torch.empty((3, B, Ncp, maxp), dtype=torch.int32, device=dev)
        lists_f = torch.empty((2, B, Ncp, maxp), dtype=torch.float32, device=dev)
        rowcol, colrow, colcnt = lists_i[0], lists_i[1], lists_i[2].view(-1)[: B * Ncp + 1]
        rowdot, coldot = lists_f[0], lists_f[1]
        overflow = colcnt[B * Ncp:]
        bitsR = bitsC = None
        if need_grad:
            bitsR = torch.empty((B, Ncp // 32, Ncp), dtype=torch.int32, device=dev)
            bitsC = torch.empty((B, Ncp // 32, Ncp), dtype=torch.int32, device=dev)
        planes = None
        if engine == "fp32":
            nneg = lib.ssp_desc_dense_simt_nblocks(B, Nc)
        else:
            nneg = lib.ssp_desc_dense_tc_nblocks(B, Nc)
            PA = torch.empty((2 if split else 1, B, Ncp, Dch), dtype=torch.bfloat16, device=dev)
            PB = torch.empty_like(PA)
            Ahi, Alo = PA[0], (PA[1] if split else None)
            Bhi, Blo = PB[0], (PB[1] if split else None)
        neg_part = torch.empty((nneg, 2), dtype=torch.float64, device=dev)
        out8 = torch.empty((8,), dtype=torch.float32, device=dev)
        if split:
            call("ssp_desc_pack2_geometry", ptr(Dc), ptr(Dwc), B, Dch, Hc, Wc, ptr(Ahi), ptr(Alo), ptr(Bhi), ptr(Blo), *geom_args, st)
            call("ssp_desc_pos_fwd_planes", ptr(Ahi), ptr(Alo), ptr(Bhi), ptr(Blo), ptr(wpts), ptr(mv_pad), B, Hc, Wc, cell,
                 dist, lamda, mpos, mneg, ptr(pos_part), ptr(rowcol), ptr(rowdot), ptr(colcnt), ptr(colrow), ptr(coldot), st)
            call("ssp_desc_dense_fwd_tc", ptr(Ahi), ptr(Alo), ptr(Bhi), ptr(Blo), ptr(mv_pad), ptr(mvbits), B, Hc, Wc, mneg,
                 ptr(neg_part), ptr(bitsR), None, ptr(debug_S), st)
            planes = (Ahi, Alo, Bhi, Blo)
        else:
            if engine != "fp32":
                call("ssp_desc_pack2_geometry", ptr(Dc), ptr(Dwc), B, Dch, Hc, Wc, ptr(Ahi), None, ptr(Bhi), None, *geom_args, st)
            with _Fork(dev) as fork:
                call("ssp_desc_pos_fwd", ptr(Dc), ptr(Dwc), ptr(wpts), ptr(mv_pad), B, Hc, Wc, Dch, cell, dist, lamda, mpos,
                     mneg, ptr(pos_part), ptr(rowcol), ptr(rowdot), ptr(colcnt), ptr(colrow), ptr(coldot), stream_of(Dc))
            if engine == "fp32":
                call("ssp_desc_dense_fwd_simt", ptr(Dc), ptr(Dwc), ptr(mv_pad), B, Hc, Wc, Dch, mneg, ptr(neg_part),
                     ptr(bitsR), ptr(bitsC), ptr(debug_S), st)
            else:
                call("ssp_desc_dense_fwd_tc", ptr(Ahi), None, ptr(Bhi), None, ptr(mv_pad), ptr(mvbits), B, Hc, Wc, mneg,
                     ptr(neg_part), ptr(bitsR), None, ptr(debug_S), st)
                planes = (Ahi, None, Bhi, None)
            fork.join()

        if step_total is not None:
            det_out, lam_loss, total = step_total[:3]
            if len(step_total) > 3 and step_total[3] is not None:
                step_total[3].join()
            call("ssp_desc_finalize", ptr(pos_part), npos, ptr(neg_part), nneg, ptr(mv_part), nmv, B, Hc, Wc, ptr(overflow),
                 ptr(out8), ptr(det_out[0]), ptr(det_out[1]), float(lam_loss), ptr(total), st)
        else:
            call("ssp_desc_finalize", ptr(pos_part), npos, ptr(neg_part), nneg, ptr(mv_part), nmv, B, Hc, Wc, ptr(overflow),
                 ptr(out8), None, None, 0.0, None, st)
        if CHECK_LIST_OVERFLOW and int(overflow[0]) != 0:
            raise RuntimeError("descriptor_loss: %d positive pairs overflowed the sparse lists" % int(overflow[0]))
        if dist_group is not None:
            from .dist import globalize_descriptor
            globalize_descriptor(out8, B, Hc, Wc, dist_group)

        if need_grad:
            ctx.save_for_backward(Dc, Dwc, mv_pad, bitsR, bitsC, lists_i, lists_f,
                                  *([p for p in planes if p is not None] if planes else []))
            ctx.out8 = out8
        ctx.meta = (B, Dch, Hc, Wc, cell, lamda, dist, mpos, engine, planes is not None and planes[1] is not None)
        ctx.fold_alpha = fold_alpha
        ctx.mark_non_differentiable(wpts)
        return out8[0], out8[1], out8[2], wpts

    @staticmethod
    @once_differentiable
    def backward(ctx, g_loss, g_pos, g_neg, _g_wpts):
        saved = ctx.saved_tensors
        Dc, Dwc, mv_pad, bitsR, bitsC, lists_i, lists_f = saved[:7]
        out8 = ctx.out8
        B, Dch, Hc, Wc, cell, lamda, dist, mpos, engine, split = ctx.meta
        dev = Dc.device
        Nc = Hc * Wc
        Ncp = _nc_pad(Nc)
        st = stream_of(Dc)
        tc_engine = engine != "fp32"
        fold = tc_engine and getattr(ctx, "fold_alpha", False)
        gscale, gmode = 1.0, 0
        if g_pos is _SAME:
            lam = float(getattr(ctx, "gscale", 1.0))
            if fold:
                g3, gscale, gmode = g_loss, lam, 1
            else:
                key = (dev.index, lam)
                if key not in _lam3:
                    _lam3[key] = torch.tensor([lam, 0.0, 0.0], dtype=torch.float32, device=dev)
                g3 = g_loss * _lam3[key]
        else:
            zero = torch.zeros((), dtype=torch.float32, device=dev)
            g3 = torch.stack([(g if g is not None else zero).reshape(()).to(torch.float32) for g in (g_loss, g_pos, g_neg)])
            g3 = g3.contiguous()
        alpha = torch.empty((B, Ncp), dtype=torch.float32, device=dev)
        srow = torch.empty((B, Ncp), dtype=torch.float32, device=dev) if fold else None
        if not fold:
            call("ssp_desc_alpha", ptr(mv_pad), ptr(g3), ptr(out8), B, Ncp, ptr(alpha), None, st)
        rowcol, colrow, colcnt = lists_i[0], lists_i[1], lists_i[2]
        rowdot, coldot = lists_f[0], lists_f[1]
        coefs = torch.empty((2,) + tuple(rowdot.shape), dtype=torch.float32, device=dev)
        colrow_sorted = torch.empty_like(colrow)
        dD = torch.empty_like(Dc)
        dDw = torch.empty_like(Dwc)
        if tc_engine:
            if split:
                Ahi, Alo, Bhi, Blo = saved[7:11]
            else:
                (Ahi, Bhi), Alo, Blo = saved[7:9], None, None
            if not fold:
                PS = torch.empty((2 if split else 1, B, Ncp, Dch), dtype=torch.bfloat16, device=dev)
                Shi, Slo = PS[0], (PS[1] if split else None)
        if fold:
            det_job = getattr(ctx, "det_job", None)
            if det_job is not None:
                x0, t0, m0, x1, t1, m1, dout, dg, d0, d1 = det_job
                call("ssp_step_bwd_prologue", ptr(x0), ptr(t0), ptr(m0), ptr(x1), ptr(t1), ptr(m1), B, Hc, Wc, ptr(dout[0]),
                     ptr(dout[1]), ptr(dg), ptr(d0), ptr(d1),
                     ptr(rowcol), ptr(rowdot), ptr(colcnt), ptr(colrow), ptr(coldot), ptr(bitsR), ptr(mv_pad), ptr(g3), gscale,
                     gmode, ptr(out8), lamda, mpos, ptr(coefs[0]), ptr(colrow_sorted), ptr(coefs[1]), ptr(alpha), ptr(srow),
                     ptr(bitsC), st)
            else:
                call("ssp_desc_pos_coef", ptr(rowcol), ptr(rowdot), ptr(colcnt), ptr(colrow), ptr(coldot), ptr(bitsR),
                     ptr(mv_pad), ptr(g3), gscale, gmode, ptr(out8), B, Ncp, lamda, mpos, ptr(coefs[0]), ptr(colrow_sorted),
                     ptr(coefs[1]), ptr(alpha), ptr(srow), ptr(bitsC), Nc, st)
            call("ssp_desc_bits_gemm_tc_pair",
                 ptr(bitsR), ptr(Bhi), ptr(Blo), ptr(srow), ptr(rowcol), ptr(coefs[0]), ptr(Bhi), ptr(Blo), ptr(dD),
                 ptr(bitsC), ptr(Ahi), ptr(Alo), ptr(alpha), ptr(colrow_sorted), ptr(coefs[1]), ptr(Ahi), ptr(Alo), ptr(dDw),
                 B, Nc, st)
        elif tc_engine:
            with _Fork(dev) as f1:
                call("ssp_desc_pos_coef", ptr(rowcol), ptr(rowdot), ptr(colcnt), ptr(colrow), ptr(coldot), ptr(bitsR),
                     ptr(mv_pad), ptr(g3), gscale, gmode, ptr(out8), B, Ncp, lamda, mpos, ptr(coefs[0]), ptr(colrow_sorted),
                     ptr(coefs[1]), None, None, ptr(bitsC), Nc, stream_of(Dc))
            call("ssp_desc_pack", ptr(Dwc), ptr(alpha), B, Dch, Nc, ptr(Shi), ptr(Slo), st)
            f1.join()
            call("ssp_desc_bits_gemm_tc_pair",
                 ptr(bitsR), ptr(Shi), ptr(Slo), None, ptr(rowcol), ptr(coefs[0]), ptr(Bhi), ptr(Blo), ptr(dD),
                 ptr(bitsC), ptr(Ahi), ptr(Alo), ptr(alpha), ptr(colrow_sorted), ptr(coefs[1]), ptr(Ahi), ptr(Alo), ptr(dDw),
                 B, Nc, st)
        else:
            with _Fork(dev) as f1:
                call("ssp_desc_pos_coef", ptr(rowcol), ptr(rowdot), ptr(colcnt), ptr(colrow), ptr(coldot), ptr(bitsR),
                     ptr(mv_pad), ptr(g3), gscale, gmode, ptr(out8), B, Ncp, lamda, mpos, ptr(coefs[0]), ptr(colrow_sorted),
                     ptr(coefs[1]), None, None, None, 0, stream_of(Dc))
            call("ssp_desc_bits_gemm_simt", ptr(bitsR), ptr(Dwc), ptr(alpha), None, None, None, None, B, Dch, Nc, ptr(dD), st)
            call("ssp_desc_bits_gemm_simt", ptr(bitsC), ptr(Dc), None, ptr(alpha), None, None, None, B, Dch, Nc, ptr(dDw), st)
            f1.join()
            call("ssp_desc_pos_apply", ptr(rowcol), ptr(coefs[0]), ptr(colrow_sorted), ptr(coefs[1]), ptr(Dc), ptr(Dwc), B, Dch, Nc, 0,
                 ptr(dD), ptr(dDw), st)
        return dD, dDw, None, None, None, None, None, None, None, None, None, None


class _Ctx(object):

    def __init__(self, needs):
        self.needs_input_grad = needs
        self.saved_tensors = ()

    def save_for_backward(self, *tensors):
        self.saved_tensors = tensors

    def mark_non_differentiable(self, *tensors):
        pass


_lam3 = {}


class LossStepFn(torch.autograd.Function):

    @staticmethod
    def forward(ctx, semi, labels_2D, mask_2D, semi_w, warped_labels, mask_warp_2D, desc, desc_w, Hm, lamda_d, dist,
                lambda_loss, engine, dist_group=None):
        c1 = _Ctx((ctx.needs_input_grad[0], False, False, ctx.needs_input_grad[3], False, False, False, False))
        B, _, Hc, Wc = semi.shape
        dev = semi.device
        fork = _Fork(dev)
        with fork:
            l0, l1, _cm = DetectorLossPairFn.forward(c1, semi, labels_2D, mask_2D, semi_w, warped_labels, mask_warp_2D, True)
        mw = f32c(mask_warp_2D.detach(), dev)
        if mw.numel() != B * Hc * Wc * 64:
            raise RuntimeError("loss_step: mask_warp_2D must be [B,1,%d,%d]" % (Hc * 8, Wc * 8))
        c2 = _Ctx((ctx.needs_input_grad[6], ctx.needs_input_grad[7]) + (False,) * 8)
        total = torch.empty((1,), dtype=torch.float32, device=dev)
        ld, pos, neg, _wpts = DescriptorLossFn.forward(c2, desc, desc_w, Hm, ("2d", mw), 8, lamda_d, dist, engine,
                                                       None, None, True, (c1.out, lambda_loss, total, fork))
        if dist_group is not None:
            from .dist import get_exchange
            get_exchange(dist_group).run(det0=c1.out[0], det1=c1.out[1], desc8=c2.out8, B_local=B, Hc=Hc, Wc=Wc,
                                         lambda_loss=lambda_loss, total=total)
        loss = total[0]
        ctx.c1, ctx.c2, ctx.lambda_loss = c1, c2, float(lambda_loss)
        ctx.mark_non_differentiable(l0, l1, ld, pos, neg)
        ctx.set_materialize_grads(False)
        return loss, l0, l1, ld, pos, neg

    @staticmethod
    @once_differentiable
    def backward(ctx, g, *_unused):
        if g is None:
            return (None,) * 14
        dev = g.device
        g = f32c(g.reshape(1), dev)
        d0 = d1 = dD = dDw = None
        want_det = ctx.needs_input_grad[0] or ctx.needs_input_grad[3]
        want_desc = ctx.needs_input_grad[6] or ctx.needs_input_grad[7]
        c2 = ctx.c2
        c2.det_job = None
        merged = (want_det and want_desc and getattr(c2, "fold_alpha", False) and c2.meta[8] != "fp32" and ctx.c1.fused2d)
        if merged:
            x0, t0, m0, x1, t1, m1 = ctx.c1.saved_tensors
            d0, d1 = torch.empty_like(x0), torch.empty_like(x1)
            c2.det_job = (x0, t0, m0, x1, t1, m1, ctx.c1.out, g, d0, d1)
        elif want_det:
            d0, _, _, d1 = DetectorLossPairFn.backward(ctx.c1, g, _SAME, None)[:4]
        if want_desc:
            c2.gscale = ctx.lambda_loss
            dD, dDw = DescriptorLossFn.backward(c2, g, _SAME, None, None)[:2]
            c2.det_job = None
        return d0, None, None, d1, None, None, dD, dDw, None, None, None, None, None, None


class SparseLossStepFn(torch.autograd.Function):

    @staticmethod
    def forward(ctx, semi, labels_2D, mask_2D, semi_w, warped_labels, mask_warp_2D, desc, desc_w, ia, ib, M, K, lamda_d,
                lambda_loss):
        from .sparse import SparseDescriptorLossFn
        c1 = _Ctx((ctx.needs_input_grad[0], False, False, ctx.needs_input_grad[3], False, False, False, False))
        l0, l1, _cm = DetectorLossPairFn.forward(c1, semi, labels_2D, mask_2D, semi_w, warped_labels, mask_warp_2D, True)
        c2 = _Ctx((ctx.needs_input_grad[6], ctx.needs_input_grad[7]) + (False,) * 6)
        ld, pos, neg = SparseDescriptorLossFn.forward(c2, desc, desc_w, ia, ib, K, ia.shape[1] - K, lamda_d)
        total = torch.empty((1,), dtype=torch.float32, device=semi.device)
        call("ssp_sparse_finalize", ptr(M), M.shape[0], ptr(c2.out3), ptr(c1.out[0]), ptr(c1.out[1]), float(lambda_loss),
             ptr(total), stream_of(total))
        ctx.c1, ctx.c2, ctx.lambda_loss = c1, c2, float(lambda_loss)
        ctx.mark_non_differentiable(l0, l1, ld, pos, neg)
        ctx.set_materialize_grads(False)
        return total[0], l0, l1, ld, pos, neg

    @staticmethod
    @once_differentiable
    def backward(ctx, g, *_unused):
        from .sparse import sparse_loss_backward
        if g is None:
            return (None,) * 14
        dev = g.device
        g = f32c(g.reshape(1), dev)
        d0 = d1 = dD = dDw = None
        if ctx.needs_input_grad[0] or ctx.needs_input_grad[3]:
            d0, _, _, d1 = DetectorLossPairFn.backward(ctx.c1, g, _SAME, None)[:4]
        if ctx.needs_input_grad[6] or ctx.needs_input_grad[7]:
            key = (dev.index, ctx.lambda_loss)
            if key not in _lam3:
                _lam3[key] = torch.tensor([ctx.lambda_loss, 0.0, 0.0], dtype=torch.float32, device=dev)
            dD, dDw = sparse_loss_backward(ctx.c2, g * _lam3[key])
        return d0, None, None, d1, None, None, dD, dDw, None, None, None, None, None, None


class LazyPairMask(object):

    def __init__(self, wpts, B, Hc, Wc, cell, dist):
        self._wpts, self._geom, self._t = wpts, (B, Hc, Wc, cell, dist), None

    @property
    def shape(self):
        B, Hc, Wc, _, _ = self._geom
        return torch.Size((B, Hc, Wc, Hc, Wc))

    def materialize(self):
        if self._t is None:
            B, Hc, Wc, cell, dist = self._geom
            m = torch.empty((B, Hc * Wc, Hc * Wc), dtype=torch.float32, device=self._wpts.device)
            call("ssp_desc_pair_mask", ptr(self._wpts), B, Hc, Wc, cell, dist, ptr(m), stream_of(m))
            self._t = m.view(B, Hc, Wc, Hc, Wc)
        return self._t

    def __getattr__(self, name):
        return getattr(self.materialize(), name)

    @classmethod
    def __torch_function__(cls, func, types, args=(), kwargs=None):
        conv = lambda a: a.materialize() if isinstance(a, LazyPairMask) else a
        return func(*[conv(a) for a in args], **{k: conv(v) for k, v in (kwargs or {}).items()})
```

Measured before the change: 142,700.

## Route sparse bit tiles in descriptor backward to a SIMT gather kernel

The dense forward kernel now counts set bits per tile while writing bitsR and stores the counts in a tile_nnz array. In the backward pass, a new SIMT kernel sums these counts per output row block. Blocks at or below a threshold (default 1024) are computed directly by gathering the selected bf16 hi/lo descriptor cells and adding the positive-pair terms. The other blocks go into a compact list that the tcgen05 bits-GEMM kernel now walks instead of every tile. The goal is to skip tensor-core work on mostly empty hinge masks, at the cost of an extra launch, a serial list-building block, and a possible slowdown if the masks turn out dense.

```diff
diff --git a/include/ssp_b200.h b/include/ssp_b200.h
--- a/include/ssp_b200.h
+++ b/include/ssp_b200.h
@@ -89,7 +89,7 @@
 int ssp_desc_dense_tc_nblocks(int B, int Nc);
 int ssp_desc_dense_fwd_tc(const void* Ahi, const void* Alo, const void* Bhi, const void* Blo, const float* mv_pad,
                           const uint32_t* mvbits , int B, int Hc, int Wc, float mneg, double* partials,
-                          uint32_t* bitsR, uint32_t* bitsC, float* dbgS, void* stream);
+                          uint32_t* bitsR, uint32_t* bitsC, int* tile_nnz , float* dbgS, void* stream);
 int ssp_desc_finalize(const double* pos_part, int npos, const double* neg_part, int nneg, const double* mv_part,
                       int nmv, int B, int Hc, int Wc, const int* overflow, float* out8,
                       const float* det0 , const float* det1, float lambda_loss, float* total , void* stream);
@@ -117,12 +117,14 @@
                             int Dch, int Nc, float* out , void* stream);
 int ssp_desc_bits_gemm_tc_planes(const uint32_t* bits, const void* Bhi, const void* Blo, const float* rowscale,
                                  const int* plist, const float* pcoef, const void* pos_hi, const void* pos_lo, int B,
-                                 int Nc, float* out , void* stream);
+                                 int Nc, float* out , const int* tile_nnz , int* scratch,
+                                 int max_sparse_nnz, void* stream);
 int ssp_desc_bits_gemm_tc_pair(const uint32_t* bits0, const void* Bhi0, const void* Blo0, const float* rowscale0,
                                const int* plist0, const float* pcoef0, const void* pos_hi0, const void* pos_lo0,
                                float* out0, const uint32_t* bits1, const void* Bhi1, const void* Blo1,
                                const float* rowscale1, const int* plist1, const float* pcoef1, const void* pos_hi1,
-                               const void* pos_lo1, float* out1, int B, int Nc, void* stream);
+                               const void* pos_lo1, float* out1, int B, int Nc, const int* tile_nnz ,
+                               int* scratch, int max_sparse_nnz, void* stream);
 
 size_t ssp_sem_ce_ws_bytes(int B, int C, int H, int W, int upsampled);
 int ssp_sem_ce_fwd(const float* logits , const long long* labels, int B, int C, int H, int W,
diff --git a/semantic-superpoint_b200/_lib.py b/semantic-superpoint_b200/_lib.py
--- a/semantic-superpoint_b200/_lib.py
+++ b/semantic-superpoint_b200/_lib.py
@@ -49,7 +49,7 @@
     "ssp_desc_pack2": (_I, [_P, _P, _P, _I, _I, _I, _P, _P, _P, _P, _P]),
     "ssp_desc_pack2_geometry": (_I, [_P, _P, _I, _I, _I, _I, _P, _P, _P, _P, _P, _P, _P, _I, _P, _P, _P, _P, _P]),
     "ssp_desc_dense_tc_nblocks": (_I, [_I, _I]),
-    "ssp_desc_dense_fwd_tc": (_I, [_P, _P, _P, _P, _P, _P, _I, _I, _I, _F, _P, _P, _P, _P, _P]),
+    "ssp_desc_dense_fwd_tc": (_I, [_P, _P, _P, _P, _P, _P, _I, _I, _I, _F, _P, _P, _P, _P, _P, _P]),
     "ssp_desc_finalize": (_I, [_P, _I, _P, _I, _P, _I, _I, _I, _I, _P, _P, _P, _P, _F, _P, _P]),
     "ssp_desc_pair_mask": (_I, [_P, _I, _I, _I, _I, _F, _P, _P]),
     "ssp_desc_alpha": (_I, [_P, _P, _P, _I, _I, _P, _P, _P]),
@@ -57,8 +57,8 @@
     "ssp_step_bwd_prologue": (_I, [_P] * 6 + [_I] * 3 + [_P] * 5 + [_P] * 8 + [_F, _I, _P, _F, _F] + [_P] * 7),
     "ssp_desc_pos_apply": (_I, [_P, _P, _P, _P, _P, _P, _I, _I, _I, _I, _P, _P, _P]),
     "ssp_desc_bits_gemm_simt": (_I, [_P, _P, _P, _P, _P, _P, _P, _I, _I, _I, _P, _P]),
-    "ssp_desc_bits_gemm_tc_planes": (_I, [_P, _P, _P, _P, _P, _P, _P, _P, _I, _I, _P, _P]),
-    "ssp_desc_bits_gemm_tc_pair": (_I, [_P] * 18 + [_I, _I, _P]),
+    "ssp_desc_bits_gemm_tc_planes": (_I, [_P, _P, _P, _P, _P, _P, _P, _P, _I, _I, _P, _P, _P, _I, _P]),
+    "ssp_desc_bits_gemm_tc_pair": (_I, [_P] * 18 + [_I, _I, _P, _P, _I, _P]),
     "ssp_sem_ce_ws_bytes": (_Z, [_I, _I, _I, _I, _I]),
     "ssp_sem_ce_fwd": (_I, [_P, _P, _I, _I, _I, _I, _I, _P, _P, _P, _Z, _P]),
     "ssp_sem_ce_bwd": (_I, [_P, _P, _P, _I, _I, _I, _I, _I, _P, _P, _P, _P]),
diff --git a/semantic-superpoint_b200/csrc/desc_tc.cu b/semantic-superpoint_b200/csrc/desc_tc.cu
--- a/semantic-superpoint_b200/csrc/desc_tc.cu
+++ b/semantic-superpoint_b200/csrc/desc_tc.cu
@@ -82,7 +82,7 @@
 __global__ void __launch_bounds__(FWD_THREADS, 1)
 desc_dense_fwd_tc_kernel(const __grid_constant__ CUtensorMap tmA, const __grid_constant__ CUtensorMap tmB,
                          const __grid_constant__ CUtensorMap tmBl, const float* __restrict__ mv_pad, const uint32_t* __restrict__ mvbits, DescGeom g, int n_last,
-                         double* __restrict__ partials, uint32_t* __restrict__ bitsR, float* __restrict__ dbgS) {
+                         double* __restrict__ partials, uint32_t* __restrict__ bitsR, int* __restrict__ tile_nnz, float* __restrict__ dbgS) {
   using Cfg = FwdCfg<P>;
   constexpr int NSTAGE = Cfg::NSTAGE;
   extern __shared__ uint8_t smem_raw[];
@@ -255,6 +255,7 @@
       TR(31);
       tc::fence_after_sync();
       uint64_t su2 = 0ull, sw2 = 0ull;
+      int nnz = 0;
 #pragma unroll 1
       for (int ch = ch0; ch < ch1; ++ch) {
         const int cbase = nt * BN + ch * 32;
@@ -276,6 +277,7 @@
         if (BITS) {
           if (fold) rowword &= __ldg(mvbits + (size_t)b * NW + cbase / 32);
           bitsR[((size_t)b * NW + cbase / 32) * g.Nc_pad + row] = rowword;
+          nnz += __popc(rowword);
         }
         if (dbgS && row < g.Nc) {
 #pragma unroll
@@ -291,6 +293,10 @@
       __syncwarp();
       if (lane == 0) tc::mbar_arrive_leader(t_empty + as);
       TR(32);
+      if (BITS && tile_nnz) {
+        nnz = __reduce_add_sync(0xffffffffu, nnz);
+        if (lane == 0) tile_nnz[((size_t)key * NT + nt) * 16 + cta_rank * 8 + warp] = nnz;
+      }
       float sa, sb, wa, wb;
       tc::unpack2(su2, sa, sb);
       tc::unpack2(sw2, wa, wb);
@@ -353,6 +359,8 @@
 
 struct BgJob {
   const uint32_t* bits;
+  const uint4* Bhi;
+  const uint4* Blo;
   const float* rowscale;
   const int* plist;
   const float* pcoef;
@@ -364,7 +372,7 @@
 template <int P>
 __global__ void __launch_bounds__(BG_THREADS, 1)
 desc_bits_gemm_tc_kernel(const __grid_constant__ CUtensorMap tm0, const __grid_constant__ CUtensorMap tm1, BgJob job0,
-                         BgJob job1, int njobs, int B, int Nc, int Nc_pad) {
+                         BgJob job1, int njobs, int B, int Nc, int Nc_pad, const int* __restrict__ dlist) {
   using Cfg = BgCfg<P>;
   constexpr int NS = BG_NS;
   static_assert(256 + BG_ACOLS * NS <= 512, "TMEM A ring does not fit");
@@ -385,12 +393,13 @@
   const uint32_t cta_rank = tc::cluster_ctarank();
   const bool leader = cta_rank == 0;
   const int ncluster = gridDim.x >> 1, cid = blockIdx.x >> 1;
-  const int T = B * njobs * MP * 2;
+  const int T = dlist ? 2 * __ldg(dlist) : B * njobs * MP * 2;
+  if (cid >= T) return;
   constexpr uint32_t A_COL0 = 256;
 
   auto decode = [&](int it, int& b, int& jb, int& mp, int& dh) {
     dh = it & 1;
-    int t = it >> 1;
+    int t = dlist ? __ldg(dlist + 1 + (it >> 1)) : it >> 1;
     mp = t % MP;
     t /= MP;
     jb = t % njobs;
@@ -635,6 +644,156 @@
   }
 }
 
+constexpr int SP_THREADS = 256;
+
+__device__ __forceinline__ int tile_nnz_sum_warp(const int* __restrict__ tile_nnz, int b, int jb, int m, int MP, int lane) {
+  const int4* p = reinterpret_cast<const int4*>(tile_nnz);
+  int s = 0;
+  for (int i = lane; i < 4 * MP; i += 32) {
+    const int u = i >> 2;
+    const size_t tile = jb ? ((size_t)b * MP + u) * MP + m : ((size_t)b * MP + m) * MP + u;
+    const int4 q = __ldg(p + tile * 4 + (i & 3));
+    s += q.x + q.y + q.z + q.w;
+  }
+  return __reduce_add_sync(0xffffffffu, s);
+}
+
+__device__ __forceinline__ uint32_t bits_natural(uint32_t w) {
+  auto spread = [](uint32_t x) {
+    x = (x | (x << 8)) & 0x00FF00FFu;
+    x = (x | (x << 4)) & 0x0F0F0F0Fu;
+    x = (x | (x << 2)) & 0x33333333u;
+    return (x | (x << 1)) & 0x55555555u;
+  };
+  return spread(w & 0xffffu) | (spread(w >> 16) << 1);
+}
+
+template <bool FMA>
+__device__ __forceinline__ void add_cell32(const uint4* __restrict__ hi, const uint4* __restrict__ lo, size_t o, float pf,
+                                           float (&a)[32]) {
+#pragma unroll
+  for (int u = 0; u < 4; ++u) {
+    const uint4 h = __ldg(hi + o + u);
+    const uint32_t hw[4] = {h.x, h.y, h.z, h.w};
+    uint32_t lw[4] = {0u, 0u, 0u, 0u};
+    if (lo) {
+      const uint4 l = __ldg(lo + o + u);
+      lw[0] = l.x; lw[1] = l.y; lw[2] = l.z; lw[3] = l.w;
+    }
+#pragma unroll
+    for (int i = 0; i < 4; ++i) {
+      const float e0 = __uint_as_float(hw[i] << 16) + __uint_as_float(lw[i] << 16);
+      const float e1 = __uint_as_float(hw[i] & 0xffff0000u) + __uint_as_float(lw[i] & 0xffff0000u);
+      if (FMA) {
+        a[u * 8 + 2 * i] = fmaf(pf, e0, a[u * 8 + 2 * i]);
+        a[u * 8 + 2 * i + 1] = fmaf(pf, e1, a[u * 8 + 2 * i + 1]);
+      } else {
+        a[u * 8 + 2 * i] += e0;
+        a[u * 8 + 2 * i + 1] += e1;
+      }
+    }
+  }
+}
+
+template <int P>
+__global__ void __launch_bounds__(SP_THREADS, 3)
+desc_bits_sparse_kernel(BgJob job0, BgJob job1, int njobs, int B, int Nc, int Nc_pad, const int* __restrict__ tile_nnz,
+                        int thr, int* __restrict__ dlist) {
+  __shared__ int s_wsum[SP_THREADS / 32];
+  const int warp = threadIdx.x >> 5, lane = threadIdx.x & 31;
+  const int MP = Nc_pad / (2 * BM);
+  const int t = blockIdx.x;
+  const int m = t % MP, jb = (t / MP) % njobs, b = t / MP / njobs;
+
+  if (blockIdx.x == 0) {
+    const int T = B * njobs * MP;
+    const int4* p4 = reinterpret_cast<const int4*>(tile_nnz);
+    int base = 0;
+    for (int i0 = 0; i0 < T; i0 += SP_THREADS) {
+      const int i = i0 + threadIdx.x;
+      bool dense = false;
+      if (i < T) {
+        const int ib = i / MP / njobs, ij = (i / MP) % njobs, im = i % MP;
+        int c = 0;
+#pragma unroll 4
+        for (int u = 0; u < MP; ++u) {
+          const size_t tile = ij ? ((size_t)ib * MP + u) * MP + im : ((size_t)ib * MP + im) * MP + u;
+#pragma unroll
+          for (int v = 0; v < 4; ++v) {
+            const int4 q = __ldg(p4 + tile * 4 + v);
+            c += q.x + q.y + q.z + q.w;
+          }
+        }
+        dense = c > thr;
+      }
+      const unsigned bal = __ballot_sync(0xffffffffu, dense);
+      if (lane == 0) s_wsum[warp] = __popc(bal);
+      __syncthreads();
+      int off = base, tot = 0;
+#pragma unroll
+      for (int w = 0; w < SP_THREADS / 32; ++w) {
+        off += w < warp ? s_wsum[w] : 0;
+        tot += s_wsum[w];
+      }
+      if (dense) dlist[1 + off + __popc(bal & ((1u << lane) - 1u))] = i;
+      base += tot;
+      __syncthreads();
+    }
+    if (threadIdx.x == 0) dlist[0] = base;
+  }
+  const int x0 = m * 2 * BM + warp * 32;
+  if (x0 >= Nc || tile_nnz_sum_warp(tile_nnz, b, jb, m, MP, lane) > thr) return;
+
+  const BgJob& J = jb ? job1 : job0;
+  const int row = x0 + lane;
+  const bool row_ok = row < Nc;
+  const int NW = Nc_pad / 32, NWv = (Nc + 31) / 32;
+  const uint32_t* bits = J.bits + (size_t)b * NW * Nc_pad + row;
+  const float rs = (J.rowscale && row_ok) ? J.rowscale[(size_t)b * Nc_pad + row] : 1.f;
+  const int* pl = J.plist ? J.plist + ((size_t)b * Nc_pad + row) * DESC_MAXP : nullptr;
+  const float* pcf = J.plist ? J.pcoef + ((size_t)b * Nc_pad + row) * DESC_MAXP : nullptr;
+  int npos = 0;
+  if (pl && row_ok) {
+#pragma unroll
+    for (int n = 0; n < DESC_MAXP; ++n)
+      if (pl[n] >= 0) npos = n + 1;
+  }
+  uint32_t any = 0;
+#pragma unroll 8
+  for (int kw = 0; kw < NWv; ++kw) any |= __ldg(bits + (size_t)kw * Nc_pad);
+  const bool warp_bits = __any_sync(0xffffffffu, any != 0u);
+  const size_t cell0 = (size_t)b * Nc_pad;
+#pragma unroll 1
+  for (int ch = 0; ch < KD / 32; ++ch) {
+    float val[32];
+#pragma unroll
+    for (int j = 0; j < 32; ++j) val[j] = 0.f;
+    if (warp_bits && any) {
+      for (int kw = 0; kw < NWv; ++kw) {
+        uint32_t n = bits_natural(__ldg(bits + (size_t)kw * Nc_pad));
+        while (n) {
+          const int j = __ffs(n) - 1;
+          n &= n - 1;
+          add_cell32<false>(J.Bhi, P == 2 ? J.Blo : nullptr, ((cell0 + kw * 32 + j) * KD + ch * 32) >> 3, 0.f, val);
+        }
+      }
+    }
+    if (J.rowscale) {
+#pragma unroll
+      for (int j = 0; j < 32; ++j) val[j] *= rs;
+    }
+    for (int n = 0; n < npos; ++n) {
+      const int pc = pl[n];
+      if (pc >= 0) add_cell32<true>(J.pos_hi, J.pos_lo, ((cell0 + pc) * KD + ch * 32) >> 3, pcf[n], val);
+    }
+    if (row_ok) {
+      float* o = J.out + ((size_t)b * KD + ch * 32) * Nc + row;
+#pragma unroll
+      for (int j = 0; j < 32; ++j) o[(size_t)j * Nc] = val[j];
+    }
+  }
+}
+
 typedef CUresult (*EncodeTiledFn)(CUtensorMap*, CUtensorMapDataType, cuuint32_t, void*, const cuuint64_t*,
                                   const cuuint64_t*, const cuuint32_t*, const cuuint32_t*, CUtensorMapInterleave,
                                   CUtensorMapSwizzle, CUtensorMapL2promotion, CUtensorMapFloatOOBfill);
@@ -728,10 +887,13 @@
 
 extern "C" int ssp_desc_dense_fwd_tc(const void* Ahi, const void* Alo, const void* Bhi, const void* Blo,
                                      const float* mv_pad, const uint32_t* mvbits, int B, int Hc, int Wc, float mneg,
-                                     double* partials, uint32_t* bitsR, uint32_t* bitsC, float* dbgS, void* stream) {
+                                     double* partials, uint32_t* bitsR, uint32_t* bitsC, int* tile_nnz, float* dbgS,
+                                     void* stream) {
   SSP_REQUIRE(Ahi && Bhi && mv_pad && partials, "ssp_desc_dense_fwd_tc: null pointer");
   SSP_REQUIRE((Alo == nullptr) == (Blo == nullptr), "ssp_desc_dense_fwd_tc: lo planes must both be given or both null");
   SSP_REQUIRE(!bitsC || bitsR, "ssp_desc_dense_fwd_tc: bitsC needs bitsR");
+  SSP_REQUIRE(!tile_nnz || bitsR, "ssp_desc_dense_fwd_tc: tile_nnz needs bitsR");
+  SSP_REQUIRE(((uintptr_t)tile_nnz & 15) == 0, "ssp_desc_dense_fwd_tc: tile_nnz must be 16-byte aligned");
   SSP_REQUIRE(B > 0 && B <= 65535 && Hc > 0 && Wc > 0, "ssp_desc_dense_fwd_tc: bad sizes");
   SSP_REQUIRE(mneg > 0.f, "ssp_desc_dense_fwd_tc: margin_neg must be > 0 (zero padding relies on it)");
   SSP_REQUIRE((((uintptr_t)Ahi | (uintptr_t)Bhi | (uintptr_t)Alo | (uintptr_t)Blo | (uintptr_t)mv_pad) & 15) == 0,
@@ -755,7 +917,7 @@
   do {                                                                                                           \
     if ((rc = set_smem(desc_dense_fwd_tc_kernel<PP, BB>, FwdCfg<PP>::SMEM))) return rc;                          \
     if ((rc = launch_cluster2(desc_dense_fwd_tc_kernel<PP, BB>, grid, FWD_THREADS, FwdCfg<PP>::SMEM, st, mA, mB, mL,         \
-                              mv_pad, mvbits, g, n_last, partials, bitsR, dbgS))) return rc;                     \
+                              mv_pad, mvbits, g, n_last, partials, bitsR, tile_nnz, dbgS))) return rc;           \
   } while (0)
   if (Alo) { if (bitsR) LAUNCH_FWD(2, true); else LAUNCH_FWD(2, false); }
   else     { if (bitsR) LAUNCH_FWD(1, true); else LAUNCH_FWD(1, false); }
@@ -775,8 +937,12 @@
   const void* pos_hi; const void* pos_lo; float* out;
 };
 
-static int bits_gemm_tc_launch(const BgHostJob* jobs, int njobs, int B, int Nc, void* stream) {
+static int bits_gemm_tc_launch(const BgHostJob* jobs, int njobs, int B, int Nc, const int* tile_nnz, int* scratch,
+                               int max_sparse_nnz, void* stream) {
   SSP_REQUIRE(B > 0 && Nc > 0, "ssp_desc_bits_gemm_tc: bad sizes");
+  SSP_REQUIRE(!tile_nnz || scratch, "ssp_desc_bits_gemm_tc: tile_nnz needs the scratch list");
+  SSP_REQUIRE(((uintptr_t)tile_nnz & 15) == 0 && ((uintptr_t)scratch & 3) == 0,
+              "ssp_desc_bits_gemm_tc: tile_nnz must be 16-byte and scratch 4-byte aligned");
   int Nc_pad = desc_nc_pad(Nc);
   uint64_t rows = (uint64_t)B * Nc_pad;
   CUtensorMap maps[2];
@@ -790,7 +956,7 @@
                 "ssp_desc_bits_gemm_tc: operands must be 16-byte aligned");
     SSP_REQUIRE((h.Blo == nullptr) == (jobs[0].Blo == nullptr), "ssp_desc_bits_gemm_tc: both jobs must use the same engine (lo planes)");
     if ((rc = make_planes_map3(&maps[j], h.Bhi, h.Blo, rows, KT))) return rc;
-    dj[j].bits = h.bits; dj[j].rowscale = h.rowscale; dj[j].plist = h.plist; dj[j].pcoef = h.pcoef;
+    dj[j].bits = h.bits; dj[j].Bhi = (const uint4*)h.Bhi; dj[j].Blo = (const uint4*)h.Blo; dj[j].rowscale = h.rowscale; dj[j].plist = h.plist; dj[j].pcoef = h.pcoef;
     dj[j].pos_hi = (const uint4*)h.pos_hi; dj[j].pos_lo = (const uint4*)h.pos_lo; dj[j].out = h.out;
   }
   if (njobs == 1) { maps[1] = maps[0]; dj[1] = dj[0]; }
@@ -798,14 +964,22 @@
   int nclusters = (int)std::min<long long>(items, std::max(1, ssp_num_sms() / 2));
   int grid = 2 * nclusters;
   cudaStream_t st = (cudaStream_t)stream;
+  if (tile_nnz) {
+    const long long sblocks = items / 2;
+    SSP_REQUIRE(sblocks < (1ll << 31), "ssp_desc_bits_gemm_tc: too many items");
+    if (jobs[0].Blo) desc_bits_sparse_kernel<2><<<(int)sblocks, SP_THREADS, 0, st>>>(dj[0], dj[1], njobs, B, Nc, Nc_pad, tile_nnz, max_sparse_nnz, scratch);
+    else             desc_bits_sparse_kernel<1><<<(int)sblocks, SP_THREADS, 0, st>>>(dj[0], dj[1], njobs, B, Nc, Nc_pad, tile_nnz, max_sparse_nnz, scratch);
+    SSP_CUDA_CHECK_LAUNCH("desc_bits_sparse_kernel");
+  }
+  const int* dlist = tile_nnz ? scratch : nullptr;
   if (jobs[0].Blo) {
     if ((rc = set_smem(desc_bits_gemm_tc_kernel<2>, BgCfg<2>::SMEM))) return rc;
     if ((rc = launch_cluster2(desc_bits_gemm_tc_kernel<2>, grid, BG_THREADS, BgCfg<2>::SMEM, st, maps[0], maps[1], dj[0], dj[1], njobs,
-                              B, Nc, Nc_pad))) return rc;
+                              B, Nc, Nc_pad, dlist))) return rc;
   } else {
     if ((rc = set_smem(desc_bits_gemm_tc_kernel<1>, BgCfg<1>::SMEM))) return rc;
     if ((rc = launch_cluster2(desc_bits_gemm_tc_kernel<1>, grid, BG_THREADS, BgCfg<1>::SMEM, st, maps[0], maps[1], dj[0], dj[1], njobs,
-                              B, Nc, Nc_pad))) return rc;
+                              B, Nc, Nc_pad, dlist))) return rc;
   }
   SSP_CUDA_CHECK_LAUNCH("desc_bits_gemm_tc_kernel");
   return SSP_OK;
@@ -813,17 +987,19 @@
 
 extern "C" int ssp_desc_bits_gemm_tc_planes(const uint32_t* bits, const void* Bhi, const void* Blo, const float* rowscale,
                                             const int* plist, const float* pcoef, const void* pos_hi, const void* pos_lo,
-                                            int B, int Nc, float* out, void* stream) {
+                                            int B, int Nc, float* out, const int* tile_nnz, int* scratch,
+                                            int max_sparse_nnz, void* stream) {
   BgHostJob j = {bits, Bhi, Blo, rowscale, plist, pcoef, pos_hi, pos_lo, out};
-  return bits_gemm_tc_launch(&j, 1, B, Nc, stream);
+  return bits_gemm_tc_launch(&j, 1, B, Nc, tile_nnz, scratch, max_sparse_nnz, stream);
 }
 
 extern "C" int ssp_desc_bits_gemm_tc_pair(const uint32_t* bits0, const void* Bhi0, const void* Blo0, const float* rowscale0,
                                           const int* plist0, const float* pcoef0, const void* pos_hi0, const void* pos_lo0,
                                           float* out0, const uint32_t* bits1, const void* Bhi1, const void* Blo1,
                                           const float* rowscale1, const int* plist1, const float* pcoef1, const void* pos_hi1,
-                                          const void* pos_lo1, float* out1, int B, int Nc, void* stream) {
+                                          const void* pos_lo1, float* out1, int B, int Nc, const int* tile_nnz,
+                                          int* scratch, int max_sparse_nnz, void* stream) {
   BgHostJob j[2] = {{bits0, Bhi0, Blo0, rowscale0, plist0, pcoef0, pos_hi0, pos_lo0, out0},
                     {bits1, Bhi1, Blo1, rowscale1, plist1, pcoef1, pos_hi1, pos_lo1, out1}};
-  return bits_gemm_tc_launch(j, 2, B, Nc, stream);
-}
+  return bits_gemm_tc_launch(j, 2, B, Nc, tile_nnz, scratch, max_sparse_nnz, stream);
+}
diff --git a/semantic-superpoint_b200/losses.py b/semantic-superpoint_b200/losses.py
--- a/semantic-superpoint_b200/losses.py
+++ b/semantic-superpoint_b200/losses.py
@@ -7,6 +7,7 @@
 _ENGINES = ("bf16x3", "bf16", "fp32")
 _engine = "bf16x3"
 CHECK_LIST_OVERFLOW = False
+BWD_SPARSE_MAX_NNZ = 1024
 
 
 def set_descriptor_engine(name):
@@ -244,10 +245,12 @@
         rowcol, colrow, colcnt = lists_i[0], lists_i[1], lists_i[2].view(-1)[: B * Ncp + 1]
         rowdot, coldot = lists_f[0], lists_f[1]
         overflow = colcnt[B * Ncp:]
-        bitsR = bitsC = None
+        bitsR = bitsC = tile_nnz = None
         if need_grad:
             bitsR = torch.empty((B, Ncp // 32, Ncp), dtype=torch.int32, device=dev)
             bitsC = torch.empty((B, Ncp // 32, Ncp), dtype=torch.int32, device=dev)
+            if engine != "fp32" and BWD_SPARSE_MAX_NNZ >= 0:
+                tile_nnz = torch.empty((B, Ncp // 256, Ncp // 256, 16), dtype=torch.int32, device=dev)
         planes = None
         if engine == "fp32":
             nneg = lib.ssp_desc_dense_simt_nblocks(B, Nc)
@@ -264,7 +267,7 @@
             call("ssp_desc_pos_fwd_planes", ptr(Ahi), ptr(Alo), ptr(Bhi), ptr(Blo), ptr(wpts), ptr(mv_pad), B, Hc, Wc, cell,
                  dist, lamda, mpos, mneg, ptr(pos_part), ptr(rowcol), ptr(rowdot), ptr(colcnt), ptr(colrow), ptr(coldot), st)
             call("ssp_desc_dense_fwd_tc", ptr(Ahi), ptr(Alo), ptr(Bhi), ptr(Blo), ptr(mv_pad), ptr(mvbits), B, Hc, Wc, mneg,
-                 ptr(neg_part), ptr(bitsR), None, ptr(debug_S), st)
+                 ptr(neg_part), ptr(bitsR), None, ptr(tile_nnz), ptr(debug_S), st)
             planes = (Ahi, Alo, Bhi, Blo)
         else:
             if engine != "fp32":
@@ -277,7 +280,7 @@
                      ptr(bitsR), ptr(bitsC), ptr(debug_S), st)
             else:
                 call("ssp_desc_dense_fwd_tc", ptr(Ahi), None, ptr(Bhi), None, ptr(mv_pad), ptr(mvbits), B, Hc, Wc, mneg,
-                     ptr(neg_part), ptr(bitsR), None, ptr(debug_S), st)
+                     ptr(neg_part), ptr(bitsR), None, ptr(tile_nnz), ptr(debug_S), st)
                 planes = (Ahi, None, Bhi, None)
             fork.join()
 
@@ -297,7 +300,7 @@
             globalize_descriptor(out8, B, Hc, Wc, dist_group)
 
         if need_grad:
-            ctx.save_for_backward(Dc, Dwc, mv_pad, bitsR, bitsC, lists_i, lists_f,
+            ctx.save_for_backward(Dc, Dwc, mv_pad, bitsR, bitsC, lists_i, lists_f, tile_nnz,
                                   *([p for p in planes if p is not None] if planes else []))
             ctx.out8 = out8
         ctx.meta = (B, Dch, Hc, Wc, cell, lamda, dist, mpos, engine, planes is not None and planes[1] is not None)
@@ -309,7 +312,7 @@
     @once_differentiable
     def backward(ctx, g_loss, g_pos, g_neg, _g_wpts):
         saved = ctx.saved_tensors
-        Dc, Dwc, mv_pad, bitsR, bitsC, lists_i, lists_f = saved[:7]
+        Dc, Dwc, mv_pad, bitsR, bitsC, lists_i, lists_f, tile_nnz = saved[:8]
         out8 = ctx.out8
         B, Dch, Hc, Wc, cell, lamda, dist, mpos, engine, split = ctx.meta
         dev = Dc.device
@@ -344,9 +347,11 @@
         dDw = torch.empty_like(Dwc)
         if tc_engine:
             if split:
-                Ahi, Alo, Bhi, Blo = saved[7:11]
+                Ahi, Alo, Bhi, Blo = saved[8:12]
             else:
-                (Ahi, Bhi), Alo, Blo = saved[7:9], None, None
+                (Ahi, Bhi), Alo, Blo = saved[8:10], None, None
+            bwd_list = torch.empty((1 + 2 * B * (Ncp // 256),), dtype=torch.int32, device=dev)
+            paths = (ptr(tile_nnz), ptr(bwd_list), BWD_SPARSE_MAX_NNZ) if BWD_SPARSE_MAX_NNZ >= 0 else (None, None, 0)
             if not fold:
                 PS = torch.empty((2 if split else 1, B, Ncp, Dch), dtype=torch.bfloat16, device=dev)
                 Shi, Slo = PS[0], (PS[1] if split else None)
@@ -366,7 +371,7 @@
             call("ssp_desc_bits_gemm_tc_pair",
                  ptr(bitsR), ptr(Bhi), ptr(Blo), ptr(srow), ptr(rowcol), ptr(coefs[0]), ptr(Bhi), ptr(Blo), ptr(dD),
                  ptr(bitsC), ptr(Ahi), ptr(Alo), ptr(alpha), ptr(colrow_sorted), ptr(coefs[1]), ptr(Ahi), ptr(Alo), ptr(dDw),
-                 B, Nc, st)
+                 B, Nc, *paths, st)
         elif tc_engine:
             with _Fork(dev) as f1:
                 call("ssp_desc_pos_coef", ptr(rowcol), ptr(rowdot), ptr(colcnt), ptr(colrow), ptr(coldot), ptr(bitsR),
@@ -377,7 +382,7 @@
             call("ssp_desc_bits_gemm_tc_pair",
                  ptr(bitsR), ptr(Shi), ptr(Slo), None, ptr(rowcol), ptr(coefs[0]), ptr(Bhi), ptr(Blo), ptr(dD),
                  ptr(bitsC), ptr(Ahi), ptr(Alo), ptr(alpha), ptr(colrow_sorted), ptr(coefs[1]), ptr(Ahi), ptr(Alo), ptr(dDw),
-                 B, Nc, st)
+                 B, Nc, *paths, st)
         else:
             with _Fork(dev) as f1:
                 call("ssp_desc_pos_coef", ptr(rowcol), ptr(rowdot), ptr(colcnt), ptr(colrow), ptr(coldot), ptr(bitsR),
```

Result: slower. 66340 (median of 6 runs) (-53.5%).
